# albanie/mcnCrossModalEmotions

Hardware: AMD Instinct MI355X
Metric: distillation-step samples/sec (face+audio pair) (higher is better)
Workload: dtype f32; 1 GPU; BASELINE config 4 shard: frozen resnet50 teacher fwd + VGGVox student fwd/bwd/SGD; per_gpu_batch=32, global_batch=32, face=224x224x3, teacher_batch=32, spectrogram=512x300x1, parallelism=dp1, weights=random-init (seeded), parameter_server=rccl-capi, streams=teacher one batch ahead on its own stream + wgrad side stream

## Files before the change

include/xmodal.h:

```cpp
#ifndef XMODAL_H
#define XMODAL_H
#include <stddef.h>
#ifdef __cplusplus
extern "C" {
#endif

enum {
  XM_OK = 0,
  XM_EINVAL = 1,
  XM_ENOMEM = 2,
  XM_EHIP = 3,
  XM_ETOOBIG = 4,
  XM_ENOTSUP = 5
};

enum { XM_POOL_MAX = 0, XM_POOL_AVG = 1 };
enum { XM_LOSS_SOFTMAXLOG = 0, XM_LOSS_CLASSERROR = 1 };
enum { XM_AGG_MAX = 0, XM_AGG_MEAN = 1, XM_AGG_PEAK = 2 };
enum { XM_MNR_CONVERGED = 0, XM_MNR_ITERLIMIT = 1, XM_MNR_NOTPD = 2, XM_MNR_BADINPUT = 3 };
enum { XM_ROC_OK = 0, XM_ROC_NAN = 1, XM_ROC_BADINPUT = 2 };

enum { XM_FUSE_RELU = 1, XM_BN_BATCH_MOMENTS = 2, XM_FUSE_SIGMOID = 4 };

int xm_version(void);
const char *xm_last_error(void);
int xm_device_alloc(void **ptr, size_t bytes);
int xm_device_free(void *ptr);
int xm_device_upload(void *dst_device, const void *src_host, size_t bytes);
int xm_device_download(void *dst_host, const void *src_device, size_t bytes);
int xm_device_synchronize(void);
enum { XM_EXEC_SINGLE_STREAM = 1 };
int xm_set_exec_hint(unsigned flags);
unsigned xm_get_exec_hint(void);
int xm_tune_load(const char *path);
int xm_tune_save(const char *path);
int xm_tune_entries(int *total, int *unsaved);
int xm_workspace_reserve(size_t bytes);
size_t xm_workspace_bytes(void);
int xm_workspace_reserve_stream(size_t bytes, void *stream);
unsigned long long xm_workspace_generation(void);
int xm_out_size(int in, int pad_a, int pad_b, int f, int dilate, int stride);

int xm_nnconv_forward(const float *x, int H, int W, int C, int N, const float *f, int FH, int FW,
                      int FC, int K, const float *b, float *y, int sy, int sx, int pt, int pb,
                      int pl, int pr, int dy, int dx, void *stream);
int xm_nnconv_forward_fused(const float *x, int H, int W, int C, int N, const float *f, int FH,
                            int FW, int FC, int K, const float *b, float *y, int sy, int sx,
                            int pt, int pb, int pl, int pr, int dy, int dx, const float *scale,
                            const float *shift, const float *residual, int flags, void *stream);
int xm_nnconv_forward_gated(const float *x, int H, int W, int C, int N, const float *f, int FH, int FW,
                            int FC, int K, const float *b, float *y, int sy, int sx, int pt, int pb,
                            int pl, int pr, int dy, int dx, const float *scale, const float *shift,
                            const float *gate, const float *residual, int flags, void *stream);
int xm_nnconv_forward_strided_residual(const float *x, int H, int W, int C, int N, const float *f, int FH, int FW,
                                       int FC, int K, const float *b, float *y, int sy, int sx, int pt, int pb,
                                       int pl, int pr, int dy, int dx, const float *scale, const float *shift,
                                       const float *gate, const float *residual, int res_H, int res_W, int res_sy,
                                       int res_sx, int flags, void *stream);
int xm_nnconv_forward_lattice(const float *x, int H, int W, int C, int N, const float *f, int FH, int FW, int FC, int K,
                              const float *b, float *y, int sy, int sx, int pt, int pb, int pl, int pr, int dy, int dx,
                              const float *scale, const float *shift, const float *residual, int flags, int lat_y,
                              int lat_x, void *stream);
enum { XM_CONV_F32 = 0, XM_CONV_BF16X3 = 1 };
int xm_nnconv_forward_split(const float *x, int H, int W, int C, int N, const float *f, int FH, int FW, int FC, int K,
                            const float *b, float *y, int sy, int sx, int pt, int pb, int pl, int pr, int dy, int dx,
                            const float *scale, const float *shift, const float *gate, const float *residual, int res_H,
                            int res_W, int res_sy, int res_sx, int flags, int precision, void *stream);
int xm_nnconv_split_geometry(int H, int W, int C, int N, int FH, int FW, int FC, int K, int sy, int sx, int pt, int pb,
                             int pl, int pr, int dy, int dx, int flags, int *can, int *want, int *blocks, int *launches);
int xm_nnconv_forward_moments(const float *x, int H, int W, int C, int N, const float *f, int FH, int FW,
                              int FC, int K, const float *b, float *y, int sy, int sx, int pt, int pb,
                              int pl, int pr, int dy, int dx, float epsilon, float *moments_out, void *stream);
int xm_nnconv_backward(const float *x, int H, int W, int C, int N, const float *f, int FH, int FW,
                       int FC, int K, const float *dzdy, float *dx_out, float *df_out,
                       float *db_out, int sy, int sx, int pt, int pb, int pl, int pr, int dy,
                       int dx, void *stream);
int xm_nnconv_prepare_backward(int H, int W, int C, int N, const float *f, int FH, int FW, int FC, int K,
                               int sy, int sx, int pt, int pb, int pl, int pr, int dy, int dx, void *stream);
int xm_params_changed(void);
int xm_nnconv_backward_accum(const float *x, int H, int W, int C, int N, const float *f, int FH, int FW,
                             int FC, int K, const float *dzdy, float *dx_out, float *df_out,
                             float *db_out, int sy, int sx, int pt, int pb, int pl, int pr, int dy,
                             int dx, const float *dx_accum, void *stream);
int xm_nnconv_backward_filter_bnrelupool(const float *x, int H, int W, int C, int N, int FH, int FW, int FC, int K,
                                         int sy, int sx, int pt, int pb, int pl, int pr, int dy, int dx,
                                         const float *y, const float *bn_g, const float *bn_b, const float *moments,
                                         int train, int ph, int pw, int psy, int psx, int ppt, int ppb, int ppl,
                                         int ppr, const unsigned char *argmax, const float *y_pool,
                                         const float *dzdy_pool, float *dzdf_out, float *dzdb_out, float *dg_out,
                                         float *db_out, void *stream);
int xm_nnconv_bnorm_relu_pool_forward(const float *x, int H, int W, int C, int N, const float *f, int FH, int FW, int FC,
                                      int K, const float *bias, int sy, int sx, int pt, int pb, int pl, int pr, int dy, int dx,
                                      const float *bn_g, const float *bn_b, float epsilon, const float *moments_in, int ph,
                                      int pw, int psy, int psx, int ppt, int ppb, int ppl, int ppr, double *gram,
                                      float *y_pool, unsigned char *argmax, float *moments_out, void *stream);
int xm_stem_gram(const float *x, int H, int W, int N, int FH, int FW, int sy, int sx, int pt, int pb, int pl, int pr,
                 double *gram, void *stream);
int xm_stem_gram_moments(const double *gram, const float *f, const float *b, int FH, int FW, int K, float epsilon,
                         float *moments_out, void *stream);
int xm_nnconv_backward_filter_bnrelupool_gram(const float *x, int H, int W, int C, int N, const float *f, int FH, int FW,
                                              int FC, int K, const float *bias, int sy, int sx, int pt, int pb, int pl,
                                              int pr, int dy, int dx, const float *bn_g, const float *moments, int train,
                                              int ph, int pw, int psy, int psx, int ppt, int ppb, int ppl, int ppr,
                                              const unsigned char *argmax, const float *y_pool, const float *dzdy_pool,
                                              const double *gram, float *df_out, float *dbias_out, float *dg_out,
                                              float *db_out, void *stream);

int xm_nnpool_forward(const float *x, int H, int W, int C, int N, int ph, int pw, int sy, int sx,
                      int pt, int pb, int pl, int pr, int method, float *y, void *stream);
int xm_nnpool_backward(const float *x, int H, int W, int C, int N, int ph, int pw, int sy, int sx,
                       int pt, int pb, int pl, int pr, int method, const float *dzdy, float *dx_out,
                       void *stream);

int xm_nnpool_forward_argmax(const float *x, int H, int W, int C, int N, int ph, int pw, int sy,
                             int sx, int pt, int pb, int pl, int pr, float *y, unsigned char *argmax,
                             void *stream);
int xm_nnpool_backward_argmax(const unsigned char *argmax, int H, int W, int C, int N, int ph, int pw,
                              int sy, int sx, int pt, int pb, int pl, int pr, const float *dzdy,
                              float *dx_out, void *stream);
int xm_nnpool_global_avg_backward_accum(const float *dzdy, const float *accum, float *dx_out, int H, int W, int C, int N,
                                        void *stream);

int xm_nnbnorm_forward(const float *x, int H, int W, int C, int N, const float *g, const float *b,
                       float epsilon, const float *moments_in, float *y, float *moments_out,
                       void *stream);
int xm_nnbnorm_forward_fused(const float *x, int H, int W, int C, int N, const float *g,
                             const float *b, float epsilon, const float *moments_in, float *y,
                             float *moments_out, int flags, void *stream);
int xm_nnbnorm_backward(const float *x, int H, int W, int C, int N, const float *g, const float *b,
                        const float *dzdy, float epsilon, const float *moments_in, float *dx_out,
                        float *dg_out, float *db_out, float *moments_out, void *stream);
int xm_nnbnorm_backward_fused(const float *x, const float *y, int H, int W, int C, int N,
                              const float *g, const float *b, const float *dzdy, float epsilon,
                              const float *moments_in, float *dx_out, float *dg_out, float *db_out,
                              float *moments_out, int flags, void *stream);

int xm_nnbnorm_backward_dxsum(const float *x, const float *y, int H, int W, int C, int N,
                              const float *g, const float *b, const float *dzdy, float epsilon,
                              const float *moments_in, float *dx_out, float *dg_out, float *db_out,
                              float *moments_out, float *dxsum_out, int flags, void *stream);

int xm_nnbnorm_relu_pool_forward(const float *x, int H, int W, int C, int N, const float *g,
                                 const float *b, float epsilon, const float *moments_in, int ph, int pw,
                                 int sy, int sx, int pt, int pb, int pl, int pr, float *y_pool,
                                 unsigned char *argmax, float *moments_out, void *stream);
int xm_nnbnorm_relu_pool_backward(const float *x, int H, int W, int C, int N, const float *g,
                                  const float *b, const float *moments, int train, int ph, int pw,
                                  int sy, int sx, int pt, int pb, int pl, int pr,
                                  const unsigned char *argmax, const float *y_pool, const float *dzdy_pool,
                                  float *dx_out, float *dg_out, float *db_out, float *dxsum_out, void *stream);

int xm_nnrelu(const float *x, size_t n, float leak, const float *dzdy, float *y, void *stream);
int xm_nnsigmoid(const float *x, size_t n, const float *dzdy, float *y, void *stream);
int xm_sum2(const float *a, const float *b, size_t n, int flags, float *y, void *stream);
int xm_scale_axpy(const float *x, int HW, int CN, const float *a, const float *r, int flags,
                  float *y, void *stream);
int xm_scale_backward(const float *x, int HW, int CN, const float *a, const float *dzdy,
                      float *dx_out, float *da_out, void *stream);

int xm_nndropout_forward(const float *x, size_t n, float rate, unsigned long long seed, unsigned long long offset,
                         float *y, float *mask_out, void *stream);
int xm_nndropout_apply(const float *x, const float *mask, size_t n, float *y, void *stream);

int xm_se_squeeze_bn(const float *u, int H, int W, int C, int N, const float *g, const float *b, const float *moments,
                     float *gp_out, void *stream);
int xm_scale_axpy_bn(const float *u, int H, int W, int C, int N, const float *a, const float *r, const float *g,
                     const float *b, const float *moments, int flags, float *y, void *stream);
int xm_se_tail_backward_reduce(const float *y, const float *dzdy, const float *u, int H, int W, int C, int N,
                               const float *g, const float *b, const float *moments, float *da_out, double *plane_sums,
                               void *stream);
int xm_se_tail_backward_apply(const float *y, const float *dzdy, const float *u, int H, int W, int C, int N,
                              const float *gate, const float *dgp, const float *g, const float *moments, int train,
                              const double *plane_sums, float *dz_out, float *du_out, float *dg_out, float *db_out,
                              void *stream);

int xm_nnsoftmaxt(const float *x, int HW, int C, int N, float temperature, float *y, void *stream);
int xm_nnsoftmaxt_backward(const float *x, const float *dzdy, int HW, int C, int N, float temperature,
                           float *dx, void *stream);
int xm_nnsoftmaxceloss(const float *x, const float *p, int C, int N, float temperature,
                       int logit_targets, const float *instance_weights, const float *dzdy,
                       float *y, void *stream);
#define XM_REGLOSS_EUCLIDEAN 0
#define XM_REGLOSS_HUBER 1
int xm_nnregloss(const float *x, const float *t, int E, int N, int kind, float sigma,
                 const float *instance_weights, const float *dzdy, float *y, void *stream);
int xm_nnloss(const float *x, const float *labels, int C, int N, int loss, const float *dzdy,
              float *y, void *stream);

int xm_sgd_update(float *w, float *m, const float *der, size_t n, float lr, float momentum,
                  float weight_decay, float batch, void *stream);
enum { XM_SOLVER_ADAGRAD = 0, XM_SOLVER_RMSPROP = 1, XM_SOLVER_ADADELTA = 2, XM_SOLVER_ADAM = 3, XM_SOLVER_NESTEROV = 4 };
int xm_solver_update(int kind, float *w, float *s1, float *s2, const float *der, size_t n, float lr,
                     float weight_decay, float batch, const float *coef, void *stream);
int xm_average_update(float *w, const float *der, size_t n, float lr, float denom,
                      void *stream);
int xm_scale_f32(float *x, size_t n, float a, void *stream);
int xm_comm_unique_id(void *id128);
int xm_comm_init(const void *id128, int rank, int world);
int xm_allreduce_sum_f32(float *buf, size_t n, void *stream);
int xm_parserv_push(float *buf, size_t n, void *producer_stream);
int xm_parserv_sync(void *consumer_stream);
int xm_comm_count(int *ranks);
int xm_comm_destroy(void);

int xm_spec_rownorm(const float *spec, int H, int W, int N, float *out, void *stream);
int xm_resample(const float *x, int Lx, const float *h, int Lh, int p, int q, int delay, float *y, int Ly, void *stream);
int xm_wav_batch(const float *wav, long long wav_len, const float *noise, long long noise_len, const long long *desc,
                 const float *ratio, int N, float *z, int L, void *stream);
int xm_spec_bucket_batch(const float *wav, long long wav_len, const long long *desc, int N, int rsize, const float *bank,
                         int taps, int hop, int B, float *out, void *stream);
int xm_spec_magnitude(const float *reim, int Wo, int B, int N, float *out, void *stream);
int xm_aggregate_logits(const float *frame_logits, int F_total, int E, const int *first,
                        const int *last, int N, int agg, float *out, float *max_label,
                        void *stream);
int xm_max_label(const float *x, int C, int N, float *labels, void *stream);
int xm_window_targets(const float *logits, int E, int n, const int *first, const int *last, int N, int agg, int P,
                      float *out, float *max_label, void *stream);
int xm_class_stats(const float *x, const float *labels, int C, int N, float *correct,
                   float *population, void *stream);
int xm_normalize_face(const float *rgb, int H, int W, int N, const float *avg3, float *out,
                      void *stream);
int xm_crop_resize_face(const float *src, int Hin, int Win, int N, float crop, int Ho, int Wo,
                        const float *avg3, float *out, void *stream);

int xm_mnrfit(const float *x, int p, int n, const int *labels, int k, const int *offsets, const int *rows, int nnz,
              int G, int max_iter, double tol_x, double *b_out, double *dev_out, int *iters_out, int *status_out,
              void *stream);
int xm_mnrval(const double *b, const float *x, int p, int n, int k, const int *offsets, const int *rows, int nnz, int G,
              const int *labels, double *probs_out, int *preds_out, int *conf_out, void *stream);

int xm_roc(const float *scores, int n, int E, const int *cls, const int *offsets, const int *rows, int nnz, int G,
           double *auc, long long *area, int *counts, int *status, int *perm_out, int *tp_out, void *stream);
int xm_roc_launches(void);
int xm_label_hist(const float *x, int N, int E, int sample_major, long long *bins, void *stream);

int xm_group_rows(const int *ids, int n, const int *keys, int T, int key_max, int *offsets_out, int *rows_out,
                  int *nnz_out, void *stream);
int xm_gather_rows(const float *mat, int F, int E, int row0, const int *rows, int n, float *packed, void *stream);
int xm_scatter_rows(const float *packed, int n, int E, float *mat, int F, int row0, const int *rows, void *stream);
int xm_track_peaks(const float *logits, int F, int E, const int *offsets, const int *rows, int T, int *frame_idx,
                   int *tag, float *maxed, void *stream);

int xm_nnaffinegrid(const float *A, int N, int Ho, int Wo, float *grid, void *stream);
int xm_nnaffinegrid_backward(const float *dgrid, int N, int Ho, int Wo, float *dA, void *stream);
int xm_nnbilinearsampler(const float *x, int H, int W, int C, int N, const float *grid, int Ho, int Wo, int No,
                         float *y, void *stream);
int xm_nnbilinearsampler_backward(const float *x, int H, int W, int C, int N, const float *grid, int Ho, int Wo,
                                  int No, const float *dy, float *dx, float *dgrid, void *stream);
int xm_ferplus_batch(const float *grey, int H, int W, int N, const int *flip, const float *A, int Ho, int Wo,
                     const float *avg3, float *out, void *stream);

enum { XM_JPEG_OK = 0, XM_JPEG_TRUNCATED = 1, XM_JPEG_BADCODE = 2 };
enum { XM_JPEG_DESC = 24, XM_JPEG_LANE = 4, XM_JPEG_QT_BYTES = 128, XM_JPEG_HT_BYTES = 1024, XM_JPEG_SIZES = 8 };
int xm_jpeg_plan(const unsigned char *bytes, const long long *offsets, int N, long long *desc, long long *lanes,
                 long long lanes_cap, unsigned char *tables, long long tables_cap, long long *sizes);
int xm_jpeg_decode_batch(const unsigned char *bytes, long long nbytes, const long long *desc, int N, const long long *lanes,
                         int nlanes, const unsigned char *tables, int nq, int nh, long long coef_elems,
                         long long plane_bytes, long long pixel_floats, float *pixels, float *faces, float crop, int Ho,
                         int Wo, const float *avg3, int *status, void *stream);

int xm_jpeg_decode_batch_split(const unsigned char *bytes, long long nbytes, const long long *desc, int N,
                               const long long *lanes, int nlanes, const unsigned char *tables, int nq, int nh,
                               long long coef_elems, long long plane_bytes, long long pixel_floats, float *pixels,
                               float *faces, float crop, int Ho, int Wo, const float *avg3, int *status, int seg_bytes,
                               int *rounds, void *stream);
int xm_jpeg_split_geometry(int *segments_per_pass, int *launches);

enum { XM_JPEG_SCAN = 24, XM_JPEG_PROG_SIZES = 11, XM_JPEG_MAX_SCANS = 256, XM_JPEG_MAX_LEVELS = 14 };
#define XM_JPEG_SMOOTH (1LL << 40)
enum { XM_JPEG_SCAN_SEQ = 0, XM_JPEG_SCAN_DC_FIRST = 1, XM_JPEG_SCAN_DC_REFINE = 2, XM_JPEG_SCAN_AC_FIRST = 3,
       XM_JPEG_SCAN_AC_REFINE = 4 };
int xm_jpeg_plan_prog(const unsigned char *bytes, const long long *offsets, int N, long long *desc, long long *scans,
                      long long scans_cap, long long *lanes, long long lanes_cap, unsigned char *tables, long long tables_cap,
                      long long *sizes);
int xm_jpeg_decode_batch_prog(const unsigned char *bytes, long long nbytes, const long long *desc, int N,
                              const long long *lanes, int nlanes, const unsigned char *tables, int nq, int nh,
                              long long coef_elems, long long plane_bytes, long long pixel_floats, float *pixels, float *faces,
                              float crop, int Ho, int Wo, const float *avg3, int *status, const long long *scans, int nscans,
                              int levels, int smooth, void *stream);

enum { XM_WAV_U8 = 0, XM_WAV_S16 = 1, XM_WAV_S24 = 2, XM_WAV_S32 = 3, XM_WAV_F32 = 4, XM_WAV_F64 = 5 };
enum { XM_WAV_OK = 0, XM_WAV_TRUNCATED = 1 };
enum { XM_WAV_DESC = 16, XM_WAV_SIZES = 2 };
int xm_wav_plan(const unsigned char *bytes, const long long *offsets, int N, const long long *ranges, int channel,
                long long out_base, long long *desc, long long *sizes);
int xm_wav_decode_batch(const unsigned char *bytes, long long nbytes, const long long *desc, int N, float *out,
                        long long out_floats, void *stream);

int xm_wav_plan_fs(const unsigned char *bytes, const long long *offsets, int N, const long long *ranges, int channel,
                   long long fs, long long out_base, long long *desc, long long *sizes);
int xm_wav_decode_resample_batch(const unsigned char *bytes, long long nbytes, const long long *desc, int N, float *out,
                                 long long out_floats, void *stream);
int xm_wav_resample_geometry(int *tile, int *launches);

enum { XM_PIX_DESC = 8, XM_PIX_SIZES = 2 };
enum { XM_PIX_BADCHAR = 1, XM_PIX_RANGE = 2, XM_PIX_COUNT = 4, XM_PIX_NOFIT = 8 };
int xm_pixcsv_plan(const unsigned char *bytes, long long nbytes, long long *desc, long long max_rows, long long *sizes);
int xm_pixcsv_decode_batch(const unsigned char *bytes, long long nbytes, const long long *desc, int N, int H, int W,
                           int transpose, float *out, long long out_floats, int *status, void *stream);
int xm_pixcsv_geometry(int *bytes_per_pass, int *launches);

int xm_nnnormalize_forward(const float *x, int H, int W, int C, int S, int N, float kappa, float alpha, float beta,
                           float *y, void *stream);
int xm_nnnormalize_backward(const float *x, const float *dzdy, int H, int W, int C, int S, int N, float kappa,
// ... 8 lines not shown
```

mcncrossmodalemotions_amd/_lib.py:

```python
import ctypes as C
import os

import torch

_HERE = os.path.dirname(os.path.abspath(__file__))
SO_PATH = os.environ.get("XM_LIB_PATH") or os.path.join(_HERE, "libxmodal_hip.so")

c_fp = C.c_void_p
_i, _f, _sz, _vp = C.c_int, C.c_float, C.c_size_t, C.c_void_p

SIGNATURES = {
    "xm_version": [],
    "xm_last_error": [],
    "xm_tune_load": [C.c_char_p],
    "xm_tune_save": [C.c_char_p],
    "xm_tune_entries": [C.POINTER(C.c_int), C.POINTER(C.c_int)],
    "xm_set_exec_hint": [C.c_uint],
    "xm_get_exec_hint": [],
    "xm_workspace_reserve": [_sz],
    "xm_workspace_bytes": [],
    "xm_workspace_reserve_stream": [_sz, _vp],
    "xm_workspace_generation": [],
    "xm_device_alloc": [C.POINTER(C.c_void_p), _sz],
    "xm_device_free": [_vp],
    "xm_device_upload": [_vp, _vp, _sz],
    "xm_device_download": [_vp, _vp, _sz],
    "xm_device_synchronize": [],
    "xm_out_size": [_i] * 6,
    "xm_nnconv_forward": [c_fp] + [_i] * 4 + [c_fp] + [_i] * 4 + [c_fp, c_fp] + [_i] * 8 + [_vp],
    "xm_nnconv_forward_moments": [c_fp] + [_i] * 4 + [c_fp] + [_i] * 4 + [c_fp, c_fp] + [_i] * 8 + [_f, c_fp, _vp],
    "xm_nnconv_forward_gated": [c_fp] + [_i] * 4 + [c_fp] + [_i] * 4 + [c_fp, c_fp] + [_i] * 8 +
                               [c_fp, c_fp, c_fp, c_fp, _i, _vp],
    "xm_nnconv_forward_strided_residual": [c_fp] + [_i] * 4 + [c_fp] + [_i] * 4 + [c_fp, c_fp] + [_i] * 8 +
                                          [c_fp, c_fp, c_fp, c_fp] + [_i] * 5 + [_vp],
    "xm_nnconv_forward_split": [c_fp] + [_i] * 4 + [c_fp] + [_i] * 4 + [c_fp, c_fp] + [_i] * 8 +
                               [c_fp, c_fp, c_fp, c_fp] + [_i] * 6 + [_vp],
    "xm_nnconv_split_geometry": [_i] * 17 + [C.POINTER(C.c_int)] * 4,
    "xm_nnconv_forward_lattice": [c_fp] + [_i] * 4 + [c_fp] + [_i] * 4 + [c_fp, c_fp] + [_i] * 8 +
                                 [c_fp, c_fp, c_fp, _i, _i, _i, _vp],
    "xm_nnconv_forward_fused": [c_fp] + [_i] * 4 + [c_fp] + [_i] * 4 + [c_fp, c_fp] + [_i] * 8 +
                               [c_fp, c_fp, c_fp, _i, _vp],
    "xm_nnconv_backward": [c_fp] + [_i] * 4 + [c_fp] + [_i] * 4 + [c_fp, c_fp, c_fp, c_fp] +
                          [_i] * 8 + [_vp],
    "xm_nnconv_backward_accum": [c_fp] + [_i] * 4 + [c_fp] + [_i] * 4 + [c_fp, c_fp, c_fp, c_fp] +
                                [_i] * 8 + [c_fp, _vp],
    "xm_nnconv_prepare_backward": [_i] * 4 + [c_fp] + [_i] * 12 + [_vp],
    "xm_nnconv_backward_filter_bnrelupool": [c_fp] + [_i] * 16 + [c_fp, c_fp, c_fp, c_fp] + [_i] * 9 +
                                            [c_fp, c_fp, c_fp, c_fp, c_fp, c_fp, c_fp, _vp],
    "xm_stem_gram": [c_fp] + [_i] * 11 + [_vp, _vp],
    "xm_stem_gram_moments": [_vp, c_fp, c_fp, _i, _i, _i, _f, c_fp, _vp],
    "xm_nnconv_backward_filter_bnrelupool_gram": [c_fp] + [_i] * 4 + [c_fp] + [_i] * 4 + [c_fp] + [_i] * 8 +
                                                 [c_fp, c_fp] + [_i] * 9 + [c_fp, c_fp, c_fp, _vp, c_fp, c_fp, c_fp, c_fp, _vp],
    "xm_nnconv_bnorm_relu_pool_forward": [c_fp] + [_i] * 4 + [c_fp] + [_i] * 4 + [c_fp] + [_i] * 8 + [c_fp, c_fp, _f, c_fp] +
                                         [_i] * 8 + [_vp, c_fp, c_fp, c_fp, _vp],
    "xm_params_changed": [],
    "xm_nnpool_forward": [c_fp] + [_i] * 13 + [c_fp, _vp],
    "xm_nnpool_backward": [c_fp] + [_i] * 13 + [c_fp, c_fp, _vp],
    "xm_nnpool_forward_argmax": [c_fp] + [_i] * 12 + [c_fp, c_fp, _vp],
    "xm_nnpool_backward_argmax": [c_fp] + [_i] * 12 + [c_fp, c_fp, _vp],
    "xm_nnpool_global_avg_backward_accum": [c_fp, c_fp, c_fp, _i, _i, _i, _i, _vp],
    "xm_nnbnorm_forward": [c_fp] + [_i] * 4 + [c_fp, c_fp, _f, c_fp, c_fp, c_fp, _vp],
    "xm_nnbnorm_forward_fused": [c_fp] + [_i] * 4 + [c_fp, c_fp, _f, c_fp, c_fp, c_fp, _i, _vp],
    "xm_nnbnorm_backward": [c_fp] + [_i] * 4 + [c_fp, c_fp, c_fp, _f, c_fp, c_fp, c_fp, c_fp, c_fp,
                                               _vp],
    "xm_nnbnorm_backward_fused": [c_fp, c_fp] + [_i] * 4 + [c_fp, c_fp, c_fp, _f, c_fp, c_fp, c_fp,
                                                             c_fp, c_fp, _i, _vp],
    "xm_nnbnorm_backward_dxsum": [c_fp, c_fp] + [_i] * 4 + [c_fp, c_fp, c_fp, _f, c_fp, c_fp, c_fp,
                                                             c_fp, c_fp, c_fp, _i, _vp],
    "xm_nnbnorm_relu_pool_forward": [c_fp] + [_i] * 4 + [c_fp, c_fp, _f, c_fp] + [_i] * 8 +
                                    [c_fp, c_fp, c_fp, _vp],
    "xm_nnbnorm_relu_pool_backward": [c_fp] + [_i] * 4 + [c_fp, c_fp, c_fp, _i] + [_i] * 8 +
                                     [c_fp, c_fp, c_fp, c_fp, c_fp, c_fp, c_fp, _vp],
    "xm_nndropout_forward": [c_fp, _sz, _f, C.c_ulonglong, C.c_ulonglong, c_fp, c_fp, _vp],
    "xm_nndropout_apply": [c_fp, c_fp, _sz, c_fp, _vp],
    "xm_nnrelu": [c_fp, _sz, _f, c_fp, c_fp, _vp],
    "xm_nnsigmoid": [c_fp, _sz, c_fp, c_fp, _vp],
    "xm_sum2": [c_fp, c_fp, _sz, _i, c_fp, _vp],
    "xm_scale_axpy": [c_fp, _i, _i, c_fp, c_fp, _i, c_fp, _vp],
    "xm_scale_backward": [c_fp, _i, _i, c_fp, c_fp, c_fp, c_fp, _vp],
    "xm_se_squeeze_bn": [c_fp] + [_i] * 4 + [c_fp, c_fp, c_fp, c_fp, _vp],
    "xm_scale_axpy_bn": [c_fp] + [_i] * 4 + [c_fp, c_fp, c_fp, c_fp, c_fp, _i, c_fp, _vp],
    "xm_se_tail_backward_reduce": [c_fp, c_fp, c_fp] + [_i] * 4 + [c_fp, c_fp, c_fp, c_fp, c_fp, _vp],
    "xm_se_tail_backward_apply": [c_fp, c_fp, c_fp] + [_i] * 4 + [c_fp, c_fp, c_fp, c_fp, _i, c_fp, c_fp, c_fp, c_fp, c_fp, _vp],
    "xm_nnsoftmaxt": [c_fp, _i, _i, _i, _f, c_fp, _vp],
    "xm_nnsoftmaxt_backward": [c_fp, c_fp, _i, _i, _i, _f, c_fp, _vp],
    "xm_nnregloss": [c_fp, c_fp, _i, _i, _i, _f, c_fp, c_fp, c_fp, _vp],
    "xm_nnsoftmaxceloss": [c_fp, c_fp, _i, _i, _f, _i, c_fp, c_fp, c_fp, _vp],
    "xm_nnloss": [c_fp, c_fp, _i, _i, _i, c_fp, c_fp, _vp],
    "xm_sgd_update": [c_fp, c_fp, c_fp, _sz, _f, _f, _f, _f, _vp],
    "xm_solver_update": [_i, c_fp, c_fp, c_fp, c_fp, _sz, _f, _f, _f, C.POINTER(C.c_float), _vp],
    "xm_average_update": [c_fp, c_fp, _sz, _f, _f, _vp],
    "xm_comm_unique_id": [_vp],
    "xm_comm_init": [_vp, _i, _i],
    "xm_allreduce_sum_f32": [c_fp, _sz, _vp],
    "xm_parserv_push": [c_fp, _sz, _vp],
    "xm_parserv_sync": [_vp],
    "xm_comm_count": [C.POINTER(C.c_int)],
    "xm_scale_f32": [c_fp, _sz, _f, _vp],
    "xm_comm_destroy": [],
    "xm_spec_rownorm": [c_fp, _i, _i, _i, c_fp, _vp],
    "xm_spec_magnitude": [c_fp, _i, _i, _i, c_fp, _vp],
    "xm_resample": [c_fp, _i, c_fp, _i, _i, _i, _i, c_fp, _i, _vp],
    "xm_wav_batch": [c_fp, C.c_longlong, c_fp, C.c_longlong, c_fp, c_fp, _i, c_fp, _i, _vp],
    "xm_spec_bucket_batch": [c_fp, C.c_longlong, c_fp, _i, _i, c_fp, _i, _i, _i, c_fp, _vp],
    "xm_aggregate_logits": [c_fp, _i, _i, c_fp, c_fp, _i, _i, c_fp, c_fp, _vp],
    "xm_max_label": [c_fp, _i, _i, c_fp, _vp],
    "xm_window_targets": [c_fp, _i, _i, c_fp, c_fp, _i, _i, _i, c_fp, c_fp, _vp],
    "xm_class_stats": [c_fp, c_fp, _i, _i, c_fp, c_fp, _vp],
    "xm_normalize_face": [c_fp, _i, _i, _i, C.POINTER(C.c_float), c_fp, _vp],
    "xm_crop_resize_face": [c_fp, _i, _i, _i, _f, _i, _i, C.POINTER(C.c_float), c_fp, _vp],
    "xm_nnaffinegrid": [c_fp, _i, _i, _i, c_fp, _vp],
    "xm_nnaffinegrid_backward": [c_fp, _i, _i, _i, c_fp, _vp],
    "xm_nnbilinearsampler": [c_fp] + [_i] * 4 + [c_fp] + [_i] * 3 + [c_fp, _vp],
    "xm_nnbilinearsampler_backward": [c_fp] + [_i] * 4 + [c_fp] + [_i] * 3 + [c_fp, c_fp, c_fp, _vp],
    "xm_ferplus_batch": [c_fp, _i, _i, _i, c_fp, c_fp, _i, _i, C.POINTER(C.c_float), c_fp, _vp],
    "xm_mnrfit": [c_fp, _i, _i, c_fp, _i, c_fp, c_fp, _i, _i, _i, C.c_double, c_fp, c_fp, c_fp, c_fp, _vp],
    "xm_mnrval": [c_fp, c_fp, _i, _i, _i, c_fp, c_fp, _i, _i, c_fp, c_fp, c_fp, c_fp, _vp],
    "xm_roc": [c_fp, _i, _i, c_fp, c_fp, c_fp, _i, _i, c_fp, c_fp, c_fp, c_fp, c_fp, c_fp, _vp],
    "xm_roc_launches": [],
    "xm_label_hist": [c_fp, _i, _i, _i, c_fp, _vp],
    "xm_group_rows": [c_fp, _i, c_fp, _i, _i, c_fp, c_fp, c_fp, _vp],
    "xm_gather_rows": [c_fp, _i, _i, _i, c_fp, _i, c_fp, _vp],
    "xm_scatter_rows": [c_fp, _i, _i, c_fp, _i, _i, c_fp, _vp],
    "xm_track_peaks": [c_fp, _i, _i, c_fp, c_fp, _i, c_fp, c_fp, c_fp, _vp],
    "xm_jpeg_plan": [_vp, _vp, _i, _vp, _vp, C.c_longlong, _vp, C.c_longlong, _vp],
    "xm_jpeg_decode_batch": [c_fp, C.c_longlong, c_fp, _i, c_fp, _i, c_fp, _i, _i, C.c_longlong, C.c_longlong, C.c_longlong,
                             c_fp, c_fp, _f, _i, _i, C.POINTER(C.c_float), c_fp, _vp],
    "xm_jpeg_decode_batch_split": [c_fp, C.c_longlong, c_fp, _i, c_fp, _i, c_fp, _i, _i, C.c_longlong, C.c_longlong,
                                   C.c_longlong, c_fp, c_fp, _f, _i, _i, C.POINTER(C.c_float), c_fp, _i, c_fp, _vp],
    "xm_jpeg_split_geometry": [C.POINTER(C.c_int), C.POINTER(C.c_int)],
    "xm_jpeg_plan_prog": [_vp, _vp, _i, _vp, _vp, C.c_longlong, _vp, C.c_longlong, _vp, C.c_longlong, _vp],
    "xm_jpeg_decode_batch_prog": [c_fp, C.c_longlong, c_fp, _i, c_fp, _i, c_fp, _i, _i, C.c_longlong, C.c_longlong,
                                  C.c_longlong, c_fp, c_fp, _f, _i, _i, C.POINTER(C.c_float), c_fp, c_fp, _i, _i, _i, _vp],
    "xm_wav_plan": [_vp, _vp, _i, _vp, _i, C.c_longlong, _vp, _vp],
    "xm_wav_decode_batch": [c_fp, C.c_longlong, c_fp, _i, c_fp, C.c_longlong, _vp],
    "xm_wav_plan_fs": [_vp, _vp, _i, _vp, _i, C.c_longlong, C.c_longlong, _vp, _vp],
    "xm_wav_decode_resample_batch": [c_fp, C.c_longlong, c_fp, _i, c_fp, C.c_longlong, _vp],
    "xm_wav_resample_geometry": [C.POINTER(C.c_int), C.POINTER(C.c_int)],
    "xm_pixcsv_plan": [_vp, C.c_longlong, _vp, C.c_longlong, _vp],
    "xm_pixcsv_decode_batch": [c_fp, C.c_longlong, c_fp, _i, _i, _i, _i, c_fp, C.c_longlong, c_fp, _vp],
    "xm_pixcsv_geometry": [C.POINTER(C.c_int), C.POINTER(C.c_int)],
    "xm_nnnormalize_forward": [c_fp] + [_i] * 5 + [_f, _f, _f, c_fp, _vp],
    "xm_nnnormalize_backward": [c_fp, c_fp] + [_i] * 5 + [_f, _f, _f, c_fp, _vp],
    "xm_nnnormalize_geometry": [C.POINTER(C.c_int)] * 3,
}
_RESTYPES = {"xm_get_exec_hint": C.c_uint, "xm_last_error": C.c_char_p, "xm_workspace_bytes": C.c_size_t,
             "xm_workspace_generation": C.c_ulonglong}
_DEBUG = {"xm_debug_set": [C.c_char_p, _i], "xm_debug_get": [C.c_char_p],
          "xm_prof_enable": [_i],
          "xm_prof_collect": [_i, C.POINTER(C.c_int), C.POINTER(C.c_double), C.POINTER(C.c_double),
                              C.POINTER(C.c_longlong)],
          "xm_prof_collect_bytes": [_i, C.POINTER(C.c_int), C.POINTER(C.c_double)],
          "xm_prof_kernel_name": [_i, C.c_char_p, _i]}
_SWITCHES = {"xm_debug_force_conv_cfg": "conv_cfg", "xm_debug_force_conv_splits": "conv_splits",
             "xm_debug_force_conv_halo": "conv_halo", "xm_debug_force_conv_stem": "conv_stem",
             "xm_debug_force_conv_stem3": "conv_stem3", "xm_debug_force_wgrad_patch": "wgrad_patch",
             "xm_debug_force_wgrad_patch_s2": "wgrad_patch_s2", "xm_debug_force_dgrad_s2": "dgrad_s2",
             "xm_debug_force_spec_blocks": "spec_blocks"}

_lib = None


class XmError(RuntimeError):
    def __init__(self, code, msg):
        super().__init__("xmodal error %d: %s" % (code, msg))
        self.code = code


def load():
    global _lib
    if _lib is not None:
        return _lib
    if not os.path.exists(SO_PATH):
        raise ImportError(
            "%s not found: build it with `python -m mcncrossmodalemotions_amd.build` "
            "(hipcc --offload-arch=gfx950); there is no CPU fallback" % SO_PATH)
    lib = C.CDLL(SO_PATH, mode=C.RTLD_GLOBAL)
    for name, args in list(SIGNATURES.items()) + list(_DEBUG.items()):
        fn = getattr(lib, name)
        fn.argtypes = args
        fn.restype = _RESTYPES.get(name, C.c_int)
    for name, key in _SWITCHES.items():
        setattr(lib, name, (lambda k: (lambda v: lib.xm_debug_set(k, int(v))))(key.encode()))
    lib.xm_debug_num_conv_cfgs = lambda: lib.xm_debug_get(b"num_conv_cfgs")
    lib.xm_debug_comm_force_single = lambda v: 0 if lib.xm_debug_set(b"comm_single", int(v)) > -2 else 1
    if hasattr(lib, "xm_debug_conv_cycles"):
        lib.xm_debug_conv_cycles.argtypes = [_i, C.POINTER(C.c_ulonglong), _i]
        lib.xm_debug_conv_cycles.restype = C.c_int
    _lib = lib
    return lib


def check(rc):
    if rc != 0:
        raise XmError(rc, load().xm_last_error().decode("utf-8", "replace"))
```

mcncrossmodalemotions_amd/build.py:

```python
import os
import subprocess
import sys
from concurrent.futures import ThreadPoolExecutor

HERE = os.path.dirname(os.path.abspath(__file__))
CSRC = os.path.join(HERE, "csrc")
TAG = os.environ.get("XM_BUILD_TAG", "")
OUT = os.path.join(HERE, "libxmodal_hip%s.so" % ("_" + TAG if TAG else ""))
SOURCES = ["context.cpp", "prof.cpp", "conv.hip", "conv_split.hip", "stem_pool.hip", "norm_pool.hip", "lrn.hip", "misc.hip", "spec.hip", "sampler.hip", "eval.hip", "roc.hip", "imdb.hip", "jpeg.hip", "jpeg_prog.hip", "wav.hip", "pixcsv.hip", "comm.cpp"]
HEADERS = ["xm_common.h", "fastdiv.h", "prof.h", "conv_plan.h", "stem_pool_plan.h", "conv_split_plan.h", "norm_pool_plan.h", "conv_tune.h", "wav_plan.h", "wav_resample.h", "pixcsv_plan.h", "jpeg_scan_plan.h", "jpeg_entropy.h", "conv_kernels.h", "stem_pool_kernels.h", os.path.join("..", "..", "include", "xmodal.h")]
FLAGS = ["--offload-arch=gfx950", "-O3", "-std=c++17", "-fPIC", "-Wall", "-Wno-unused-function"]
if os.environ.get("XM_DEBUG_CYCLES"):
    FLAGS.append("-DXM_DEBUG_CYCLES")
FLAGS += os.environ.get("XM_DEFINES", "").split()


def _stale(target, deps):
    if not os.path.exists(target):
        return True
    t = os.path.getmtime(target)
    return any(os.path.getmtime(d) > t for d in deps)


def build(force=False, verbose=False):
    hipcc = os.environ.get("HIPCC", "/opt/rocm/bin/hipcc")
    objdir = os.path.join(CSRC, "_obj" + ("_" + TAG if TAG else ""))
    os.makedirs(objdir, exist_ok=True)
    hdrs = [os.path.join(CSRC, h) for h in HEADERS]
    jobs = []
    objs = []
    for s in SOURCES:
        src = os.path.join(CSRC, s)
        obj = os.path.join(objdir, s + ".o")
        objs.append(obj)
        if force or _stale(obj, [src] + hdrs):
            jobs.append([hipcc] + FLAGS + ["-x", "hip", "-c", src, "-o", obj])

    def run(cmd):
        if verbose:
            print(" ".join(cmd), file=sys.stderr)
        subprocess.check_call(cmd)

    if jobs:
        with ThreadPoolExecutor(max_workers=min(len(jobs), os.cpu_count() or 4)) as ex:
            list(ex.map(run, jobs))
    if jobs or force or _stale(OUT, objs):
        run([hipcc, "--offload-arch=gfx950", "-shared", "-fPIC", "-o", OUT] + objs +
            ["-L/opt/rocm/lib", "-lrccl", "-Wl,-rpath,/opt/rocm/lib"])
    return OUT


if __name__ == "__main__":
    print(build(force="--force" in sys.argv, verbose=True))
```

mcncrossmodalemotions_amd/csrc/context.cpp:

```cpp
#include <cstdlib>
#include <map>
#include <string>
#include <vector>

#include "xm_common.h"

namespace xm {
bool path_on(Path p) {
  static const char *const kEnv[kPathCount] = {"XM_NO_HYBRID",      "XM_NO_HALO",        "XM_NO_SKINNY",     "XM_NO_SKINNY4",
                                               "XM_NO_STEM",        "XM_NO_STEM_WGRAD",  "XM_NO_DMA",        "XM_NO_FUSED_STATS",
                                               "XM_DGRAD_MERGE",    "XM_NO_FAST_TRANSPOSE", "XM_NO_POOL_LDS", "XM_NO_POOL_PATCH",
                                               "XM_NO_POOL_POOLED", "XM_NO_W8", "XM_NO_WGRAD_PATCH", "XM_NO_WGRAD_PATCH_S2", "XM_NO_DGRAD_S2", "XM_NO_STEM3"};
  static bool on[kPathCount];
  static bool read = false;
  if (!read) {
    for (int i = 0; i < kPathCount; ++i) on[i] = getenv(kEnv[i]) == nullptr;
    read = true;
  }
  return on[p];
}

long long env_int(const char *name, long long dflt) {
  const char *e = getenv(name);
  return (e && *e) ? atoll(e) : dflt;
}
double env_double(const char *name, double dflt) {
  const char *e = getenv(name);
  return (e && *e) ? atof(e) : dflt;
}

static char g_err[512] = "";
char *err_buf() { return g_err; }

int fail(int code, const char *fmt, ...) {
  va_list ap;
  va_start(ap, fmt);
  vsnprintf(g_err, sizeof g_err, fmt, ap);
  va_end(ap);
  return code;
}

struct WsBuf {
  void *ptr = nullptr;
  size_t cap = 0;
};
static std::map<hipStream_t, WsBuf> g_ws;
static unsigned long long g_ws_generation = 0;

int ws_get(size_t bytes, void **ptr, hipStream_t stream) {
  WsBuf &w = g_ws[stream];
  if (bytes > w.cap) {
    size_t want = bytes + bytes / 4 + (1u << 20);
    static const bool verbose = getenv("XM_WS_VERBOSE") != nullptr;
    if (verbose) fprintf(stderr, "[xm ws] stream %p grow %zu -> %zu\n", (void *)stream, w.cap, want);
    ++g_ws_generation;
    if (w.ptr) {
      hipError_t e = hipDeviceSynchronize();
      if (e != hipSuccess) return fail(XM_EHIP, "hipDeviceSynchronize -> %s", hipGetErrorString(e));
      (void)hipFree(w.ptr);
      w.ptr = nullptr;
      w.cap = 0;
    }
    hipError_t e = hipMalloc(&w.ptr, want);
    if (e != hipSuccess) {
      w.ptr = nullptr;
      return fail(XM_ENOMEM, "workspace hipMalloc(%zu) -> %s", want, hipGetErrorString(e));
    }
    w.cap = want;
  }
  *ptr = w.ptr;
  return XM_OK;
}

static std::map<std::string, void *> g_tables;

const void *cached_device_table(const void *host, size_t bytes) {
  std::string key((const char *)host, bytes);
  auto it = g_tables.find(key);
  if (it != g_tables.end()) return it->second;
  void *d = nullptr;
  static const bool verbose = getenv("XM_WS_VERBOSE") != nullptr;
  if (verbose) fprintf(stderr, "[xm ws] new device table %zu bytes (#%zu)\n", bytes, g_tables.size());
  if (hipMalloc(&d, bytes) != hipSuccess) return nullptr;
  if (hipMemcpy(d, host, bytes, hipMemcpyHostToDevice) != hipSuccess) {
    (void)hipFree(d);
    return nullptr;
  }
  g_tables.emplace(std::move(key), d);
  return d;
}

}

extern "C" {

int xm_version(void) { return 124; }
const char *xm_last_error(void) { return xm::err_buf(); }

int xm_workspace_reserve(size_t bytes) {
  void *p;
  return xm::ws_get(bytes, &p, nullptr);
}
int xm_workspace_reserve_stream(size_t bytes, void *stream) {
  void *p;
  return xm::ws_get(bytes, &p, (hipStream_t)stream);
}
unsigned long long xm_workspace_generation(void) { return xm::g_ws_generation; }

int xm_device_alloc(void **ptr, size_t bytes) {
  if (!ptr) return xm::fail(XM_EINVAL, "device_alloc: NULL output");
  *ptr = nullptr;
  if (bytes == 0) return XM_OK;
  hipError_t e = hipMalloc(ptr, bytes);
  if (e != hipSuccess) return xm::fail(XM_ENOMEM, "hipMalloc(%zu) -> %s", bytes, hipGetErrorString(e));
  return XM_OK;
}
int xm_device_free(void *ptr) {
  if (!ptr) return XM_OK;
  hipError_t e = hipFree(ptr);
  if (e != hipSuccess) return xm::fail(XM_EHIP, "hipFree -> %s", hipGetErrorString(e));
  return XM_OK;
}
int xm_device_upload(void *dst_device, const void *src_host, size_t bytes) {
  if (bytes == 0) return XM_OK;
  if (!dst_device || !src_host) return xm::fail(XM_EINVAL, "device_upload: NULL pointer");
  hipError_t e = hipMemcpy(dst_device, src_host, bytes, hipMemcpyHostToDevice);
  if (e != hipSuccess) return xm::fail(XM_EHIP, "hipMemcpy(H2D, %zu) -> %s", bytes, hipGetErrorString(e));
  return XM_OK;
}
int xm_device_download(void *dst_host, const void *src_device, size_t bytes) {
  if (bytes == 0) return XM_OK;
  if (!dst_host || !src_device) return xm::fail(XM_EINVAL, "device_download: NULL pointer");
  hipError_t e = hipMemcpy(dst_host, src_device, bytes, hipMemcpyDeviceToHost);
  if (e != hipSuccess) return xm::fail(XM_EHIP, "hipMemcpy(D2H, %zu) -> %s", bytes, hipGetErrorString(e));
  return XM_OK;
}
int xm_device_synchronize(void) {
  hipError_t e = hipDeviceSynchronize();
  if (e != hipSuccess) return xm::fail(XM_EHIP, "hipDeviceSynchronize -> %s", hipGetErrorString(e));
  return XM_OK;
}
size_t xm_workspace_bytes(void) {
  size_t t = 0;
  for (auto &kv : xm::g_ws) t += kv.second.cap;
  return t;
}

int xm_out_size(int in, int pad_a, int pad_b, int f, int dilate, int stride) {
  return xm::out_size(in, pad_a, pad_b, f, dilate, stride);
}
}
```

mcncrossmodalemotions_amd/csrc/conv.hip:

```cpp
#include <dlfcn.h>

#include <algorithm>
#include <climits>
#include <cstdlib>
#include <map>
#include <string>
#include <vector>

#include "conv_kernels.h"
#include "conv_tune.h"
#include "prof.h"

namespace xm {


__global__ void pad_filter_kernel(const float *__restrict__ f, float *__restrict__ o, int M, int R,
                                  int Rp) {
  size_t i = blockIdx.x * (size_t)blockDim.x + threadIdx.x;
  if (i >= (size_t)M * Rp) return;
  int r = (int)(i % Rp);
  size_t m = i / Rp;
  o[i] = r < R ? f[m * R + r] : 0.f;
}

// ... 969 lines not shown
  a.A = f, a.lda = R, a.nbm = 1, a.nbn = (a.NP + 127) / 128, a.slab = nullptr;
  a.hyS = 1, a.hyFull = 0, a.hyTps = 0, a.hyP0 = 0, a.piReal = 0;
  a.dbgCycles = g_dbg_cycles;
  const double abytes = (double)a.xBytes + 4.0 * a.M * a.Rtrue + 4.0 * a.M * (double)a.NP;
  ProfScope ps(prof_key(kProfStem), 2.0 * a.M * (double)a.NP * a.Rtrue, st, abytes);
  const int grid = stem_grid(a.NP);
  if (a.gsy == 2) hipLaunchKernelGGL(conv_stem_kernel<2>, dim3(grid), dim3(256), 0, st, a, a.nbn);
  else hipLaunchKernelGGL(conv_stem_kernel<1>, dim3(grid), dim3(256), 0, st, a, a.nbn);
  XM_LAUNCH_CHECK();
  return XM_OK;
}

static int g_force_stem3 = -1;
static bool stem3_ok(const ConvGemmArgs &a, const Geo &g, const float *x, bool stats) {
  if (!path_on(kPathStem3) || forced_tiling()) return false;
  if (!stem3_can(g, (uintptr_t)x, epilogue_flags(a, stats))) return false;
  return g_force_stem3 == 1 || fills_chip(g);
}
static int launch_stem3(ConvGemmArgs a, const float *f, int R, hipStream_t st) {
  a.A = f, a.lda = R, a.nbm = 1, a.nbn = a.NP / 128, a.slab = nullptr;
  const double abytes = (double)a.xBytes + 4.0 * a.M * a.Rtrue + 4.0 * a.M * (double)a.NP;
  static const bool wide_on = env_int("XM_STEM3_WIDE", 1) != 0;
  const int pij = (int)a.divPIJ.d, pi = (int)a.divPI.d;
  const bool wide = wide_on && pij % 256 == 0 && pi >= 86;
  if (wide) a.nbn = a.NP / 256;
  ProfScope ps(prof_key(kProfStem3, wide ? 1 : 0), 2.0 * a.M * (double)a.NP * a.Rtrue, st, abytes);
  const int grid = std::min(512, (a.nbn + 7) / 8 * 8);
  if (wide) hipLaunchKernelGGL(conv_stem3_kernel<2>, dim3(grid), dim3(256), 0, st, a, a.nbn);
  else hipLaunchKernelGGL(conv_stem3_kernel<1>, dim3(grid), dim3(256), 0, st, a, a.nbn);
  XM_LAUNCH_CHECK();
  return XM_OK;
}

static size_t slab_floats(int M, int NP, int Rp, int ncfg, int nU, int nV, int Rtrue) {
  ConvGemmArgs proto{};
  proto.M = M, proto.NP = NP, proto.Rp = Rp;
  size_t need = 0;
  for (int c = 0; c < ncfg; ++c) {
    int sp;
    need = std::max(need, gemm_slab_floats(proto, c, &sp));
  }
  if (nU <= 3 && nV <= 3 && nU * nV >= 4 && Rtrue % (kHaloCB * nU * nV) == 0) {
    proto.Rtrue = Rtrue, proto.nU = nU, proto.nV = nV;
    need = std::max(need, halo_slab_floats(proto));
  }
  return need;
}

struct FwdOperands {
  const float *x, *A, *b, *scale, *shift, *resid, *gate;
  float *y;
  const int2 *taps;
  int lda, Rp, relu;
  bool bigTaps, dma_ok;
  int rH = 0, rW = 0, rsy = 1, rsx = 1;
  bool resid_strided(const Geo &g) const { return resid && (rH != g.Ho || rW != g.Wo || rsy != 1 || rsx != 1); }
};

static ConvGemmArgs forward_args(const Geo &g, int grp, const FwdOperands &o) {
  ConvGemmArgs a{};
  const size_t xoff = (size_t)grp * g.FC * g.H * g.W, yoff = (size_t)grp * g.Kg * g.Ho * g.Wo;
  a.A = o.A + (size_t)grp * g.Kg * o.lda, a.lda = o.lda, a.aBytes = (unsigned)((size_t)g.Kg * o.lda * 4);
  a.X = o.x + xoff, a.xBytes = (unsigned)((x_elements(g) - xoff) * 4), a.xSampleStride = g.H * g.W * g.C;
  a.Y = o.y + yoff, a.taps = o.taps, a.tapStride = (unsigned)((size_t)g.H * g.W * 4);
  a.bias = o.b ? o.b + grp * g.Kg : nullptr;
  a.scale = o.scale ? o.scale + grp * g.Kg : nullptr, a.shift = o.shift ? o.shift + grp * g.Kg : nullptr;
  a.resid = o.resid ? o.resid + yoff : nullptr, a.relu = o.relu;
  if (o.resid_strided(g)) {
    a.resid = o.resid + (size_t)grp * g.Kg * o.rH * o.rW;
    a.rsOn = 1, a.rsy = o.rsy, a.rsx = o.rsx, a.rH = o.rH;
    a.rChanStride = o.rH * o.rW, a.rSampleStride = o.rH * o.rW * g.K;
  }
  a.gate = o.gate ? o.gate + (size_t)grp * g.Kg : nullptr, a.gateStride = g.K;
  a.M = g.Kg, a.Rp = o.Rp, a.Rtrue = g.R;
  a.PI = g.Ho, a.PJ = g.Wo, a.NP = g.Ho * g.Wo * g.N;
  a.divPIJ = make_fastdiv((uint32_t)(g.Ho * g.Wo)), a.divPI = make_fastdiv((uint32_t)g.Ho);
  a.gsy = g.sy, a.gsx = g.sx, a.gh0 = -g.pt, a.gw0 = -g.pl, a.LimH = g.H, a.LimW = g.W;
  a.nU = o.bigTaps ? 1 : g.FH, a.nV = o.bigTaps ? 1 : g.FW;
  a.du0 = 0, a.dus = g.dy, a.dv0 = 0, a.dvs = g.dx;
  a.osy = 1, a.osx = 1, a.oh0 = 0, a.ow0 = 0, a.OH = g.Ho;
  a.oChanStride = g.Ho * g.Wo, a.oSampleStride = g.Ho * g.Wo * g.K, a.divMU = make_fastdiv(1), a.oUStride = 0;
  a.vecStore = ((g.Ho * g.Wo) % 4 == 0 && (((uintptr_t)a.Y | (a.rsOn ? 0 : (uintptr_t)a.resid)) & 15) == 0) ? 1 : 0;
  a.dmaOk = (o.dma_ok && a.vecStore && !a.rsOn) ? 1 : 0;
  return a;
}

struct FwdStats {
  bool ok;
  float *part;
  int ncg;
};
static ConvGemmArgs stats_args(const ConvGemmArgs &a, FwdStats &s, int ncg) {
  ConvGemmArgs aa = a;
  s.ncg = ncg;
  if (ncg > 0) aa.statPart = s.part, aa.statNcg = ncg;
  return aa;
}
static int forward_stats_reduce(const FwdStats &s, double *part2, float *moments_out, int K, int NP, float eps, hipStream_t st) {
  const int S = std::max(1, std::min(64, s.ncg / 768));
  g_last_stats_splits = S;
  hipLaunchKernelGGL(conv_stats_reduce_kernel, dim3((K + 7) / 8, S), dim3(256), 0, st, s.part, moments_out, part2, K, s.ncg, S,
                     (double)NP, eps);
  XM_LAUNCH_CHECK();
  if (S > 1) {
    hipLaunchKernelGGL(conv_stats_finalize2_kernel, dim3((K + 255) / 256), dim3(256), 0, st, part2, moments_out, K, S,
                       (double)NP, eps);
    XM_LAUNCH_CHECK();
  }
  return XM_OK;
}

static int forward_run(const Geo &g, const ConvGemmArgs &a, const float *x, const float *f, int mode, float *slab,
                       FwdStats &s, hipStream_t st) {
  auto gemm = [&](int ci) {
    int sp;
    ci = a.dmaOk ? ci : base_cfg(ci);
    gemm_slab_floats(a, ci, &sp);
    const bool carry = s.ok && sp == 1 && g_force_splits <= 1;
    ConvGemmArgs aa = stats_args(a, s, carry ? (a.NP + kCfgs[ci].bn() - 1) / kCfgs[ci].bn() : 0);
    const int rc_ = launch_gemm(aa, mode, ci, sp, slab, st);
    if (aa.statPart) s.ncg = aa.statNcg;
    return rc_;
  };
  const TuneKey key = tune_key_forward(0, g, a.M, a.NP, a.Rp, mode + (s.ok ? 4 : 0));
  const int ci = tune_cfg(key, pick_cfg(a.M, a.NP, a.Rp / kBK), st, gemm, a.dmaOk ? kNumCfg : kNumBaseCfg, w8_skip(a.M, a.NP));
  if (!a.rsOn && stem_ok(a, g, x, s.ok)) {
    auto arm = [&](int h) { return h ? launch_stem(stats_args(a, s, s.ok ? stem_grid(a.NP) : 0), f, g.R, st) : gemm(ci); };
    return arm(select_arm(7, key, st, 2, kOneChallenger, kHaloMargin, g_force_stem, arm));
  }
  if (!a.rsOn && stem3_ok(a, g, x, s.ok)) {
    auto arm = [&](int h) { return h ? launch_stem3(a, f, g.R, st) : gemm(ci); };
    return arm(select_arm(12, key, st, 2, kOneChallenger, kHaloMargin, g_force_stem3, arm));
  }
  ConvGemmArgs ah = a;
  const int hneed = (forced_tiling() || a.rsOn) ? 0 : halo_setup(ah, g.N);
  const bool hok[4] = {true, halo_var_ok(ah, hneed, 0), halo_var_ok(ah, hneed, 1), halo_var_ok(ah, hneed, 2)};
  auto arm = [&](int h) {
    if (!h) return gemm(ci);
    const bool carry = s.ok && halo_splits(ah, h - 1) == 1;
    return launch_halo(stats_args(ah, s, carry ? (a.NP + 127) / 128 : 0), h - 1, slab, st);
  };
  return arm(select_arm(4, key, st, 4, hok, kHaloMargin, halo_forced(hok), arm));
}

static bool fwd_dma_ok(const Geo &g, const float *x, const float *f, bool need_pad, int mode) {
  return !need_pad && mode == 0 && g.FH == 1 && g.FW == 1 && g.sy == 1 && g.sx == 1 && g.dy == 1 &&
         g.dx == 1 && (g.H * g.W) % 4 == 0 && ((uintptr_t)x & 15) == 0 && ((uintptr_t)f & 15) == 0 &&
         g.R % kBK == 0 && path_on(kPathDma);
}

static int conv_forward(const float *x, const float *f, const float *b, float *y, const Geo &g,
                        const float *scale, const float *shift, const float *resid, int relu,
                        hipStream_t st, float *moments_out = nullptr, float eps = 0.f, const float *gate = nullptr,
                        int res_H = 0, int res_W = 0, int res_sy = 1, int res_sx = 1) {
  const bool padded = (g.pt | g.pb | g.pl | g.pr) != 0;
  const bool bigTaps = g.FH * g.FW > 63;
  if (bigTaps && padded)
    return fail(XM_ENOTSUP, "vl_nnconv: padded filters with more than 63 spatial taps (%dx%d) are not built",
                g.FH, g.FW);
  const int Rp = (g.R + kBK - 1) / kBK * kBK;
  const bool need_pad = (g.R % kBK) != 0 || ((uintptr_t)f & 15);
  const int mode = (padded || Rp != g.R) ? 1 : 0;
  const int NP = g.Ho * g.Wo * g.N;
  const size_t slabf = slab_floats(g.Kg, NP, Rp, kNumCfg, g.FH, g.FW, g.R);
  const bool dma_ok = fwd_dma_ok(g, x, f, need_pad, mode);
  const bool want_stats = moments_out != nullptr && g.G == 1 && path_on(kPathFusedStats);
  const size_t statf = want_stats ? (size_t)2 * g.K * std::max((NP + 31) / 32, stem_grid(NP)) : 0;
  const size_t stat2 = want_stats ? (size_t)2 * g.K * 64 : 0;
  WsCarver ws;
  int rc = ws.init(WsCarver::need(need_pad ? (size_t)g.K * Rp : 0, 4) + WsCarver::need(slabf, 4) +
                       WsCarver::need(statf, 4) + WsCarver::need(stat2, 8), st);
  if (rc) return rc;
  FwdOperands o{x, f, b, scale, shift, resid, gate, y, device_taps(fwd_tap_table(g, Rp, bigTaps)), g.R, Rp, relu, bigTaps, dma_ok};
  if (!o.taps) return fail(XM_ENOMEM, "vl_nnconv: tap table allocation failed");
  if (resid) o.rH = res_H > 0 ? res_H : g.Ho, o.rW = res_W > 0 ? res_W : g.Wo, o.rsy = res_sy, o.rsx = res_sx;
  if (need_pad) {
    float *Ap = ws.take<float>((size_t)g.K * Rp);
    size_t n = (size_t)g.K * Rp;
    hipLaunchKernelGGL(pad_filter_kernel, dim3((unsigned)((n + 255) / 256)), dim3(256), 0, st, f, Ap,
                       g.K, g.R, Rp);
    XM_LAUNCH_CHECK();
    o.A = Ap;
    o.lda = Rp;
  }
  float *slab = slabf ? ws.take<float>(slabf) : nullptr;
  float *statp = statf ? ws.take<float>(statf) : nullptr;
  double *statp2 = stat2 ? ws.take<double>(stat2) : nullptr;
  bool stats_done = false;
  if (moments_out) g_last_stats_splits = 0;
  for (int grp = 0; grp < g.G; ++grp) {
    ConvGemmArgs a = forward_args(g, grp, o);
    FwdStats s{want_stats && a.vecStore && !relu && !resid, statp, 0};
    if (s.ok) a.dmaOk = 0;
    rc = forward_run(g, a, x, f, mode, slab, s, st);
    if (rc) return rc;
    if (s.ncg > 0) {
      rc = forward_stats_reduce(s, statp2, moments_out, g.K, NP, eps, st);
      if (rc) return rc;
      stats_done = true;
    }
  }
  if (moments_out && !stats_done) return bn_batch_moments(y, g.Ho, g.Wo, g.K, g.N, eps, moments_out, st);
  return XM_OK;
}

struct FullExtentPlan {
  int ci;
  int tps;
  int hyS, hyTps, hyP0;
};
static int g_last_lattice = 0;

static bool full_extent_plan(const Geo &g, const ConvGemmArgs &a, const float *x, int mode, bool have_slab, hipStream_t st,
                             FullExtentPlan &p) {
  if (stem_ok(a, g, x, false) || stem3_ok(a, g, x, false)) return false;
  const TuneKey key = tune_key_forward(0, g, a.M, a.NP, a.Rp, mode);
  int ci = pick_cfg(a.M, a.NP, a.Rp / kBK);
  const int ncfg = a.dmaOk ? kNumCfg : kNumBaseCfg;
  if (g_force_cfg >= 0) ci = g_force_cfg < ncfg ? g_force_cfg : base_cfg(g_force_cfg);
  else if (tune_must_measure(key, st, &ci)) return false;
  ConvGemmArgs ah = a;
  const int hneed = forced_tiling() ? 0 : halo_setup(ah, g.N);
  const bool hok[4] = {true, halo_var_ok(ah, hneed, 0), halo_var_ok(ah, hneed, 1), halo_var_ok(ah, hneed, 2)};
  if (hok[1] || hok[2] || hok[3]) {
    int arm = halo_forced(hok);
    if (arm < 0) {
      TuneKey k4 = key;
      k4.kind = 4;
      arm = 0;
      if (tune_must_measure(k4, st, &arm)) return false;
      if (arm < 0 || arm >= 4 || !hok[arm]) arm = 0;
    }
    if (arm != 0) return false;
  }
  ci = a.dmaOk ? ci : base_cfg(ci);
  int sp;
  gemm_slab_floats(a, ci, &sp);
  if (ci == kCfgW8 && !path_on(kPathW8)) ci = 0;
  const Cfg &c = kCfgs[ci];
  ConvGemmArgs t = a;
  t.nbm = (a.M + c.bm() - 1) / c.bm(), t.nbn = (a.NP + c.bn() - 1) / c.bn(), t.nkt = a.Rp / kBK;
  t.statPart = nullptr;
  p.tps = (t.nkt + sp - 1) / sp;
  p.hyS = 1, p.hyTps = 0, p.hyP0 = 0;
  if (p.tps >= t.nkt && have_slab) {
    int full;
    const int hyS = hybrid_plan(t, ci, &full);
    if (hyS > 1) {
      p.hyTps = (t.nkt + hyS - 1) / hyS;
      p.hyS = (t.nkt + p.hyTps - 1) / p.hyTps;
      p.hyP0 = full / t.nbm * c.bn();
    }
  }
  p.ci = !is_dma_cfg(ci) ? ci : (kCfgs[ci].tm * kCfgs[ci].tn == 1 ? 3 : base_cfg(ci));
  return true;
}

static int launch_gemm_lattice(ConvGemmArgs a, int mode, int ci, int tps, float *slab, int p0, hipStream_t st) {
  const Cfg &c = kCfgs[ci];
  a.nbm = (a.M + c.bm() - 1) / c.bm();
  a.nbn = (a.NP + c.bn() - 1) / c.bn();
  a.nkt = a.Rp / kBK;
  a.tilesPerSplit = std::min(tps, a.nkt);
  const int splits = (a.nkt + a.tilesPerSplit - 1) / a.tilesPerSplit;
  a.NPs = (a.NP + 3) & ~3;
  a.slab = splits > 1 ? slab : nullptr;
  a.dbgCycles = g_dbg_cycles;
  a.hyS = 1, a.hyFull = 0, a.hyTps = 0, a.hyP0 = 0;
  if (splits > 1 && !slab) return fail(XM_EINVAL, "vl_nnconv(lattice): split launch without a slab");
  {
    const double abytes = (double)a.xBytes + 4.0 * a.M * a.Rtrue + 4.0 * a.M * (double)a.NP;
    ProfScope ps(prof_key(kProfGemm, ci * 2 + mode), 2.0 * a.M * (double)a.NP * a.Rtrue, st, abytes);
    const dim3 grid(a.nbm * a.nbn, splits);
    if (mode) launch_gemm_cfg<1>(ci, a, grid, st);
    else launch_gemm_cfg<0>(ci, a, grid, st);
  }
  XM_LAUNCH_CHECK();
  g_last_combine = 0;
  if (splits > 1) {
    a.slab += p0, a.hyP0 = p0;
    launch_splitk_epilogue(a, splits, a.NP - p0, false, st);
    g_last_combine = -splits;
    XM_LAUNCH_CHECK();
  }
  return XM_OK;
}

static int conv_forward_lattice(const float *x, const float *f, const float *b, float *y, const Geo &g, const float *scale,
                                const float *shift, int relu, int ly, int lx, hipStream_t st, int *ran) {
  *ran = 0;
  const bool padded = (g.pt | g.pb | g.pl | g.pr) != 0;
  const bool bigTaps = g.FH * g.FW > 63;
  if (bigTaps && padded) return XM_OK;
  if (g.G != 1) return XM_OK;
  const int Rp = (g.R + kBK - 1) / kBK * kBK;
  const bool need_pad = (g.R % kBK) != 0 || ((uintptr_t)f & 15);
  const int mode = (padded || Rp != g.R) ? 1 : 0;
  const int NP = g.Ho * g.Wo * g.N;
  const bool have_slab = slab_floats(g.Kg, NP, Rp, kNumCfg, g.FH, g.FW, g.R) > 0;
  const int PI = lattice_extent(g.Ho, ly), PJ = lattice_extent(g.Wo, lx), NPl = PI * PJ * g.N;
  FwdOperands o{x, f, b, scale, shift, nullptr, nullptr, y, nullptr, g.R, Rp, relu, bigTaps, fwd_dma_ok(g, x, f, need_pad, mode)};
  FullExtentPlan p;
  if (!full_extent_plan(g, forward_args(g, 0, o), x, mode, have_slab, st, p)) return XM_OK;
  const int nkt = Rp / kBK;
  const int z = p.hyS > 1 ? p.hyS : (nkt + p.tps - 1) / p.tps;
  const long long cut = p.hyS > 1 ? lattice_pixels_below(p.hyP0, g.Ho, g.Wo, ly, lx) : 0;
  const int n0 = (int)(cut / (PI * PJ));
  const int NPz = NPl - n0 * PI * PJ;
  const size_t slabf = z > 1 ? (size_t)z * g.Kg * ((NPz + 3) & ~3) : 0;
  WsCarver ws;
  int rc = ws.init(WsCarver::need(need_pad ? (size_t)g.K * Rp : 0, 4) + WsCarver::need(slabf, 4), st);
  if (rc) return rc;
  o.taps = device_taps(fwd_tap_table(g, Rp, bigTaps));
  if (!o.taps) return fail(XM_ENOMEM, "vl_nnconv: tap table allocation failed");
  if (need_pad) {
    float *Ap = ws.take<float>((size_t)g.K * Rp);
    const size_t n = (size_t)g.K * Rp;
    hipLaunchKernelGGL(pad_filter_kernel, dim3((unsigned)((n + 255) / 256)), dim3(256), 0, st, f, Ap, g.K, g.R, Rp);
    XM_LAUNCH_CHECK();
    o.A = Ap;
    o.lda = Rp;
  }
  float *slab = slabf ? ws.take<float>(slabf) : nullptr;
  for (int grp = 0; grp < g.G; ++grp) {
    ConvGemmArgs a = forward_args(g, grp, o);
    a.PI = PI, a.PJ = PJ, a.NP = NPl;
    a.divPIJ = make_fastdiv((uint32_t)(PI * PJ)), a.divPI = make_fastdiv((uint32_t)PI);
    a.gsy = g.sy * ly, a.gsx = g.sx * lx;
    a.osy = ly, a.osx = lx;
    a.vecStore = 0, a.dmaOk = 0;
    if (p.hyS <= 1) {
      rc = launch_gemm_lattice(a, mode, p.ci, p.tps, slab, 0, st);
      if (rc) return rc;
      continue;
    }
    if (cut > 0) {
      ConvGemmArgs a1 = a;
      a1.NP = (int)cut;
      rc = launch_gemm_lattice(a1, mode, p.ci, nkt, nullptr, 0, st);
      if (rc) return rc;
    }
    if (cut < NPl) {
      ConvGemmArgs a2 = a;
      const size_t xskip = (size_t)n0 * g.H * g.W * g.C;
      a2.X += xskip, a2.xBytes -= (unsigned)(xskip * 4), a2.Y += (size_t)n0 * a.oSampleStride;
      a2.NP = NPz;
      rc = launch_gemm_lattice(a2, mode, p.ci, p.hyTps, slab, (int)(cut - (long long)n0 * PI * PJ), st);
      if (rc) return rc;
    }
  }
  *ran = 1;
  return XM_OK;
}

struct PrepKey {
// ... 561 lines not shown
    *s->value = s->normalise(value);
    return old;
  }
  if (key && strcmp(key, "comm_single") == 0) return comm_force_single(value);
  return INT_MIN;
}
int xm_debug_get(const char *key) {
  if (key && strcmp(key, "num_conv_cfgs") == 0) return kNumCfg;
  if (key && strcmp(key, "conv_last_combine") == 0) return g_last_combine;
  if (key && strcmp(key, "conv_last_lattice") == 0) return g_last_lattice;
  if (key && strcmp(key, "wgrad_last_splits") == 0) return g_last_wgrad_splits;
  if (key && strcmp(key, "bias_grad_last_splits") == 0) return g_last_bias_splits;
  if (key && strcmp(key, "stats_last_splits") == 0) return g_last_stats_splits;
  if (key && strcmp(key, "dgrad_last_transpose") == 0) return g_last_dgrad_transpose;
  if (key && strcmp(key, "dgrad_last_prepared") == 0) return g_last_dgrad_prepared;
  const DebugSwitch *s = debug_switch(key);
  return s ? *s->value : INT_MIN;
}

int xm_set_exec_hint(unsigned flags) {
  if (flags & ~(unsigned)XM_EXEC_SINGLE_STREAM) return fail(XM_EINVAL, "xm_set_exec_hint: unknown flag bits 0x%x", flags);
  g_exec_hint = flags;
  return XM_OK;
}
unsigned xm_get_exec_hint(void) { return g_exec_hint; }


int xm_tune_load(const char *path) {
  return g_tune.load(path && path[0] ? path : tune_default_path().c_str());
}
int xm_tune_save(const char *path) {
  tune_load_once();
  const std::string p = path && path[0] ? std::string(path) : tune_default_path();
  const int rc = g_tune.save(p.c_str());
  if (rc == 1) return fail(XM_EINVAL, "xm_tune_save: cannot write %s.tmp", p.c_str());
  if (rc) return fail(XM_EINVAL, "xm_tune_save: rename to %s failed", p.c_str());
  return XM_OK;
}
int xm_tune_entries(int *total, int *unsaved) {
  tune_load_once();
  if (total) *total = g_tune.size();
  if (unsaved) *unsaved = g_tune.unsaved;
  return XM_OK;
}
#ifdef XM_DEBUG_CYCLES
int xm_debug_conv_cycles(int on, unsigned long long *out, int nblocks) {
  const size_t bytes = 4096 * 4 * sizeof(unsigned long long);
  if (on && !g_dbg_cycles) {
    if (hipMalloc((void **)&g_dbg_cycles, bytes) != hipSuccess) return XM_ENOMEM;
    (void)hipMemset(g_dbg_cycles, 0, bytes);
  }
  if (out && g_dbg_cycles)
    (void)hipMemcpy(out, g_dbg_cycles, (size_t)std::min(nblocks, 4096) * 32, hipMemcpyDeviceToHost);
  if (!on && g_dbg_cycles) {
    (void)hipFree(g_dbg_cycles);
    g_dbg_cycles = nullptr;
  }
  return XM_OK;
}
#endif

static int fused_forward(const float *x, int H, int W, int C, int N, const float *f, int FH, int FW,
                         int FC, int K, const float *b, float *y, int sy, int sx, int pt, int pb,
                         int pl, int pr, int dy, int dx, const float *scale, const float *shift,
                         const float *gate, const float *residual, int res_H, int res_W, int res_sy,
                         int res_sx, int flags, void *stream) {
  Geo g;
  int rc = make_geo(g, H, W, C, N, FH, FW, FC, K, sy, sx, pt, pb, pl, pr, dy, dx);
  if (rc) return rc;
  if (res_H == 0) res_H = g.Ho, res_W = g.Wo, res_sy = res_sx = 1;
  if (!x || !f || !y) return fail(XM_EINVAL, "vl_nnconv: NULL tensor");
  if ((scale == nullptr) != (shift == nullptr))
    return fail(XM_EINVAL, "vl_nnconv(fused): scale and shift must be given together");
  if ((flags & XM_FUSE_RELU) && (flags & XM_FUSE_SIGMOID))
    return fail(XM_EINVAL, "vl_nnconv(fused): relu and sigmoid are exclusive");
  if (gate && (flags & XM_FUSE_SIGMOID)) return fail(XM_ENOTSUP, "vl_nnconv(gated): sigmoid epilogue is not built");
  if (residual) {
    if (res_sy < 1 || res_sx < 1 || res_H < 1 || res_W < 1 || g.Ho != (res_H - 1) / res_sy + 1 ||
        g.Wo != (res_W - 1) / res_sx + 1)
      return fail(XM_EINVAL, "vl_nnconv(fused): a %d x %d residual sampled with stride [%d %d] does not give the %d x %d output",
                  res_H, res_W, res_sy, res_sx, g.Ho, g.Wo);
    if ((long long)res_H * res_W * g.K * g.N >= (1LL << 30))
      return fail(XM_ETOOBIG, "vl_nnconv(fused): residual with >= 2^30 elements (4 GiB)");
  }
  hipStream_t st = (hipStream_t)stream;
  if (!gate && !residual && fc_skinny_ok(g))
    return fc_skinny_forward(x, f, b, y, g, (flags & XM_FUSE_SIGMOID) ? 2 : ((flags & XM_FUSE_RELU) ? 1 : 0), st, scale,
                             shift);
  rc = conv_forward(x, f, b, y, g, scale, shift, residual, (flags & XM_FUSE_RELU) ? 1 : 0, st, nullptr, 0.f, gate, res_H,
                    res_W, res_sy, res_sx);
  if (rc || !(flags & XM_FUSE_SIGMOID)) return rc;
  return xm_nnsigmoid(y, (size_t)g.Ho * g.Wo * g.K * g.N, nullptr, y, stream);
}

int xm_nnconv_forward_fused(const float *x, int H, int W, int C, int N, const float *f, int FH,
                            int FW, int FC, int K, const float *b, float *y, int sy, int sx,
                            int pt, int pb, int pl, int pr, int dy, int dx, const float *scale,
                            const float *shift, const float *residual, int flags, void *stream) {
  return fused_forward(x, H, W, C, N, f, FH, FW, FC, K, b, y, sy, sx, pt, pb, pl, pr, dy, dx, scale, shift, nullptr, residual,
                       0, 0, 1, 1, flags, stream);
}

int xm_nnconv_forward_strided_residual(const float *x, int H, int W, int C, int N, const float *f, int FH, int FW,
                                       int FC, int K, const float *b, float *y, int sy, int sx, int pt, int pb,
                                       int pl, int pr, int dy, int dx, const float *scale, const float *shift,
                                       const float *gate, const float *residual, int res_H, int res_W, int res_sy,
                                       int res_sx, int flags, void *stream) {
  if (residual && res_H < 1) return fail(XM_EINVAL, "vl_nnconv(fused): residual extent must be positive");
  return fused_forward(x, H, W, C, N, f, FH, FW, FC, K, b, y, sy, sx, pt, pb, pl, pr, dy, dx, scale, shift, gate, residual,
                       residual ? res_H : 0, res_W, res_sy, res_sx, flags, stream);
}

int xm_nnconv_forward_lattice(const float *x, int H, int W, int C, int N, const float *f, int FH, int FW, int FC, int K,
                              const float *b, float *y, int sy, int sx, int pt, int pb, int pl, int pr, int dy, int dx,
                              const float *scale, const float *shift, const float *residual, int flags, int lat_y,
                              int lat_x, void *stream) {
  Geo g;
  int rc = make_geo(g, H, W, C, N, FH, FW, FC, K, sy, sx, pt, pb, pl, pr, dy, dx);
  if (rc) return rc;
  if (!x || !f || !y) return fail(XM_EINVAL, "vl_nnconv: NULL tensor");
  if (lat_y < 1 || lat_x < 1) return fail(XM_EINVAL, "vl_nnconv(lattice): the lattice steps must be >= 1, got [%d %d]", lat_y, lat_x);
  if ((scale == nullptr) != (shift == nullptr))
    return fail(XM_EINVAL, "vl_nnconv(fused): scale and shift must be given together");
  if (residual) return fail(XM_ENOTSUP, "vl_nnconv(lattice): a residual operand is not built");
  if (flags & ~XM_FUSE_RELU) return fail(XM_ENOTSUP, "vl_nnconv(lattice): only the ReLU epilogue is built");
  g_last_lattice = 0;
  int ran = 0;
  if ((lat_y > 1 || lat_x > 1) && !fc_skinny_ok(g)) {
    rc = conv_forward_lattice(x, f, b, y, g, scale, shift, (flags & XM_FUSE_RELU) ? 1 : 0, lat_y, lat_x, (hipStream_t)stream, &ran);
    if (rc) return rc;
  }
  g_last_lattice = ran;
  if (ran) return XM_OK;
  return fused_forward(x, H, W, C, N, f, FH, FW, FC, K, b, y, sy, sx, pt, pb, pl, pr, dy, dx, scale, shift, nullptr, nullptr, 0, 0,
                       1, 1, flags, stream);
}

int xm_nnconv_forward_moments(const float *x, int H, int W, int C, int N, const float *f, int FH, int FW,
                              int FC, int K, const float *b, float *y, int sy, int sx, int pt, int pb,
                              int pl, int pr, int dy, int dx, float epsilon, float *moments_out, void *stream) {
  Geo g;
  int rc = make_geo(g, H, W, C, N, FH, FW, FC, K, sy, sx, pt, pb, pl, pr, dy, dx);
  if (rc) return rc;
  if (!x || !f || !y || !moments_out) return fail(XM_EINVAL, "vl_nnconv(+moments): NULL tensor");
  hipStream_t st = (hipStream_t)stream;
  if (fc_skinny_ok(g)) {
    g_last_stats_splits = 0;
    rc = fc_skinny_forward(x, f, b, y, g, 0, st);
    return rc ? rc : bn_batch_moments(y, g.Ho, g.Wo, g.K, g.N, epsilon, moments_out, st);
  }
  return conv_forward(x, f, b, y, g, nullptr, nullptr, nullptr, 0, st, moments_out, epsilon);
}

int xm_nnconv_forward_gated(const float *x, int H, int W, int C, int N, const float *f, int FH, int FW,
                            int FC, int K, const float *b, float *y, int sy, int sx, int pt, int pb,
                            int pl, int pr, int dy, int dx, const float *scale, const float *shift,
                            const float *gate, const float *residual, int flags, void *stream) {
  if (!gate) return fail(XM_EINVAL, "vl_nnconv(gated): NULL tensor");
  return fused_forward(x, H, W, C, N, f, FH, FW, FC, K, b, y, sy, sx, pt, pb, pl, pr, dy, dx, scale, shift, gate, residual,
                       0, 0, 1, 1, flags, stream);
}

int xm_nnconv_forward(const float *x, int H, int W, int C, int N, const float *f, int FH, int FW,
                      int FC, int K, const float *b, float *y, int sy, int sx, int pt, int pb,
                      int pl, int pr, int dy, int dx, void *stream) {
  return xm_nnconv_forward_fused(x, H, W, C, N, f, FH, FW, FC, K, b, y, sy, sx, pt, pb, pl, pr, dy,
                                 dx, nullptr, nullptr, nullptr, 0, stream);
}

int xm_nnconv_prepare_backward(int H, int W, int C, int N, const float *f, int FH, int FW, int FC, int K,
                               int sy, int sx, int pt, int pb, int pl, int pr, int dy, int dx, void *stream) {
  Geo g;
  int rc = make_geo(g, H, W, C, N, FH, FW, FC, K, sy, sx, pt, pb, pl, pr, dy, dx);
  if (rc) return rc;
  if (!f) return fail(XM_EINVAL, "vl_nnconv: F is NULL");
  return conv_dgrad(f, nullptr, nullptr, g, (hipStream_t)stream, nullptr, true);
}

int xm_params_changed(void) {
  ++g_param_version;
  return XM_OK;
}

int xm_nnconv_backward_filter_bnrelupool(const float *x, int H, int W, int C, int N, int FH, int FW, int FC, int K, int sy,
                                         int sx, int pt, int pb, int pl, int pr, int dy, int dx, const float *y,
                                         const float *bn_g, const float *bn_b, const float *moments, int train, int ph,
                                         int pw, int psy, int psx, int ppt, int ppb, int ppl, int ppr,
                                         const unsigned char *argmax, const float *y_pool, const float *dzdy_pool,
                                         float *df_out, float *dbias_out, float *dg_out, float *db_out, void *stream) {
  Geo g;
  int rc = make_geo(g, H, W, C, N, FH, FW, FC, K, sy, sx, pt, pb, pl, pr, dy, dx);
  if (rc) return rc;
  if (!x || !y || !bn_g || !bn_b || !moments || !argmax || !dzdy_pool || !df_out)
    return fail(XM_EINVAL, "vl_nnconv(filter derivative through bnorm+relu+pool): NULL tensor");
  hipStream_t st = (hipStream_t)stream;
  const int pHo = out_size(g.Ho, ppt, ppb, ph, 1, psy), pWo = out_size(g.Wo, ppl, ppr, pw, 1, psx);
  const bool ok = g_force_stem != 0 && stem_wgrad_can(g, (uintptr_t)x, (uintptr_t)y) && g.K == g.Kg && y_pool != nullptr &&
                  pool3x3s2_unpadded(ph, pw, psy, psx, ppt, ppb, ppl, ppr) && (g.Ho & 1) == 0 && pHo >= 1 && pWo >= 1 &&
                  (!dbias_out || g.R < 64) && fits_i32_bytes((size_t)pHo * pWo * g.K * g.N);
  if (!ok)
    return fail(XM_ENOTSUP, "vl_nnconv(filter derivative through bnorm+relu+pool): geometry not covered by the fused kernel");
  const int grid = stem_grid(g.Ho * g.Wo * g.N);
  WsCarver ws;
  rc = ws.init(WsCarver::need((size_t)6 * g.K, 4) + WsCarver::need((size_t)grid * 96 * 64, 4) + bnpool_sums_need(g.K, g.N), st);
  if (rc) return rc;
  float *rowc = ws.take<float>((size_t)6 * g.K);
  float *spart = ws.take<float>((size_t)grid * 96 * 64);
  rc = bnpool_backward_sums(ws, y, g.Ho, g.Wo, g.K, g.N, bn_g, bn_b, moments, train, ph, pw, psy, psx, ppt, ppb, ppl, ppr,
                            argmax, y_pool, dzdy_pool, dg_out, db_out, rowc, st);
  if (rc) return rc;
  StemBnp bnp{dzdy_pool, argmax, rowc, pHo, pWo, dbias_out};
  return launch_stem_wgrad(x, y, df_out, g, spart, grid, st, &bnp);
}

int xm_nnconv_backward(const float *x, int H, int W, int C, int N, const float *f, int FH, int FW,
                       int FC, int K, const float *dzdy, float *dx_out, float *df_out,
                       float *db_out, int sy, int sx, int pt, int pb, int pl, int pr, int dy,
                       int dx, void *stream) {
  return xm_nnconv_backward_accum(x, H, W, C, N, f, FH, FW, FC, K, dzdy, dx_out, df_out, db_out, sy, sx, pt,
                                  pb, pl, pr, dy, dx, nullptr, stream);
}

int xm_nnconv_backward_accum(const float *x, int H, int W, int C, int N, const float *f, int FH, int FW,
                             int FC, int K, const float *dzdy, float *dx_out, float *df_out,
                             float *db_out, int sy, int sx, int pt, int pb, int pl, int pr, int dy,
                             int dx, const float *dx_accum, void *stream) {
  Geo g;
  int rc = make_geo(g, H, W, C, N, FH, FW, FC, K, sy, sx, pt, pb, pl, pr, dy, dx);
  if (rc) return rc;
  if (!dzdy) return fail(XM_EINVAL, "vl_nnconv: DZDY is NULL in backward mode");
  hipStream_t st = (hipStream_t)stream;
  if (db_out) {
    int S = std::max(1, std::min(N, 2048 / K));
    if ((long long)g.Ho * g.Wo < 1024) S = 1;
    WsCarver ws;
    rc = ws.init(WsCarver::need((size_t)K * S, 8), st);
    if (rc) return rc;
    double *part = ws.take<double>((size_t)K * S);
    const int HWo = g.Ho * g.Wo;
    const bool vec = (HWo & 3) == 0 && ((uintptr_t)dzdy & 15) == 0;
    g_last_bias_splits = S;
    hipLaunchKernelGGL(bias_grad_partial_kernel, dim3(K, S), dim3(256), 0, st, dzdy, part, HWo, K, N, S, vec ? 1 : 0,
                       make_fastdiv((uint32_t)(vec ? HWo >> 2 : HWo)));
    XM_LAUNCH_CHECK();
    hipLaunchKernelGGL(bias_grad_finalize_kernel, dim3((K + 3) / 4), dim3(256), 0, st, part, db_out,
                       K, S);
    XM_LAUNCH_CHECK();
  }
  if (df_out) {
    if (!x) return fail(XM_EINVAL, "vl_nnconv: X is NULL but DZDF requested");
    rc = conv_wgrad(x, dzdy, df_out, g, st);
    if (rc) return rc;
  }
  if (dx_out) {
    if (!f) return fail(XM_EINVAL, "vl_nnconv: F is NULL but DZDX requested");
    if (dx_accum == dx_out) return fail(XM_EINVAL, "vl_nnconv: dx_accum must not alias dx_out");
    rc = conv_dgrad(f, dzdy, dx_out, g, st, dx_accum);
    if (rc) return rc;
  }
  return XM_OK;
}
}
```

mcncrossmodalemotions_amd/csrc/prof.cpp:

```cpp
#include "prof.h"

#include <algorithm>
#include <vector>

#include "xm_common.h"

namespace xm {

bool g_prof_on = false;
static std::vector<ProfRec> g_prof;
static std::vector<hipEvent_t> g_event_pool;

static hipEvent_t prof_event() {
  if (!g_event_pool.empty()) {
    hipEvent_t e = g_event_pool.back();
    g_event_pool.pop_back();
    return e;
  }
  hipEvent_t e;
  (void)hipEventCreate(&e);
  return e;
}
void prof_begin(ProfRec &r, hipStream_t st) {
  r.start = prof_event();
  r.stop = prof_event();
  (void)hipEventRecord(r.start, st);
}
void prof_end(const ProfRec &r, hipStream_t st) {
  (void)hipEventRecord(r.stop, st);
  g_prof.push_back(r);
}

struct ProfRow {
  ProfKind kind;
  int nsub;
  const char *names[6];
};
static const ProfRow kProfRows[] = {
    {kProfGemm, 2 * 12, {}},
    {kProfWgrad, 4 * 7, {}},
    {kProfGemmMulti, 2 * 8, {}},
    {kProfHalo, 3, {"conv_halo_kernel<2, 2, 2, 2, 512>", "conv_halo_kernel<3, 1, 1, 4, 512>", "conv_halo_kernel<3, 1, 1, 4, 1024>"}},
    {kProfHaloMulti, 3, {"conv_halo_multi_kernel<2, 2, 2, 2, 512>", "conv_halo_multi_kernel<3, 1, 1, 4, 512>",
                         "conv_halo_multi_kernel<3, 1, 1, 4, 1024>"}},
    {kProfStem, 1, {"conv_stem_kernel<2>"}},
    {kProfStemWgrad, 2, {"conv_stem_wgrad_kernel<2>", "conv_stem_wgrad_bnp_kernel<2, 2>"}},
    {kProfWgradPatch, 1, {"conv_wgrad_patch_kernel<30>"}},
    {kProfWgradPatchS2, 1, {"conv_wgrad_patch_s2_kernel<5, 2>"}},
    {kProfDgradS2, 1, {"conv_dgrad_s2_kernel<1>"}},
    {kProfStem3, 2, {"conv_stem3_kernel<1>", "conv_stem3_kernel<2>"}},
    {kProfStemGram, 1, {"stem_gram_kernel<2>"}},
    {kProfStemWgradPool, 2, {"conv_stem_wgrad_pool_kernel<2, false>", "conv_stem_wgrad_pool_kernel<2, true>"}},
    {kProfStemBnpoolFwd, 1, {"conv_stem_bnpool_fwd_kernel"}},
    {kProfSpec, 4, {"spec_bank_kernel", "spec_plan_kernel", "spec_gemm_kernel", "spec_finish_kernel"}},
    {kProfJpeg, 6, {"jpeg_clear_kernel", "jpeg_entropy_kernel", "jpeg_idct_kernel", "jpeg_colour_kernel",
                    "crop_resize_face_ragged_kernel", "jpeg_entropy_split_kernel"}},
    {kProfJpegProg, 3, {"jpeg_entropy_prog_kernel", "jpeg_smooth_kernel", "jpeg_smooth_dc_kernel"}},
    {kProfWav, 1, {"wav_decode_kernel"}},
    {kProfWavRate, 2, {"wav_rate_gain_kernel", "wav_resample_kernel"}},
    {kProfPixcsv, 1, {"pixcsv_decode_kernel"}},
    {kProfConvSplit, 1, {"conv_split_kernel"}},
    {kProfLrn, 6, {"lrn_forward_kernel<5, false>", "lrn_forward_kernel<5, true>", "lrn_backward_kernel<5, false>",
                   "lrn_backward_kernel<5, true>", "lrn_general_kernel<false>", "lrn_general_kernel<true>"}},
};

static size_t prof_slot(std::vector<int> &ks, int key) {
  const size_t i = std::find(ks.begin(), ks.end(), key) - ks.begin();
  if (i == ks.size()) ks.push_back(key);
  return i;
}

}

using namespace xm;

extern "C" {

int xm_prof_enable(int on) {
  if (on) {
    for (auto &r : g_prof) {
      g_event_pool.push_back(r.start);
      g_event_pool.push_back(r.stop);
    }
    g_prof.clear();
  }
  g_prof_on = on != 0;
  return XM_OK;
}

int xm_prof_collect(int cap, int *keys, double *total_ms, double *total_flops, long long *launches) {
  std::vector<int> ks;
  std::vector<double> ms, fl;
  std::vector<long long> cnt;
  for (auto &r : g_prof) {
    float t = 0.f;
    if (hipEventElapsedTime(&t, r.start, r.stop) != hipSuccess) continue;
    const size_t i = prof_slot(ks, r.key);
    if (i == ms.size()) ms.push_back(0), fl.push_back(0), cnt.push_back(0);
    ms[i] += t;
    fl[i] += r.flops;
    cnt[i] += 1;
  }
  for (size_t i = 0; i < ks.size() && (int)i < cap; ++i) {
    keys[i] = ks[i];
    total_ms[i] = ms[i];
    total_flops[i] = fl[i];
    launches[i] = cnt[i];
  }
  return (int)ks.size();
}

int xm_prof_collect_bytes(int cap, int *keys, double *total_bytes) {
  std::vector<int> ks;
  std::vector<double> by;
  for (auto &r : g_prof) {
    const size_t i = prof_slot(ks, r.key);
    if (i == by.size()) by.push_back(0);
    by[i] += r.bytes;
  }
  for (size_t i = 0; i < ks.size() && (int)i < cap; ++i) {
    keys[i] = ks[i];
    total_bytes[i] = by[i];
  }
  return (int)ks.size();
}

int xm_prof_kernel_name(int key, char *buf, int len) {
  if (!buf || len <= 0) return fail(XM_EINVAL, "xm_prof_kernel_name: no buffer");
  buf[0] = 0;
  const int kind = key / 100, sub = key % 100;
  for (const ProfRow &row : kProfRows) {
    if (key < 0 || kind != row.kind || sub >= row.nsub) continue;
    if (row.names[0]) {
      snprintf(buf, len, "%s", row.names[sub]);
      return XM_OK;
    }
    if (conv_cfg_kernel_name(row.kind, sub, buf, len)) return XM_OK;
  }
  return fail(XM_EINVAL, "xm_prof_kernel_name: no launch site records key %d", key);
}

}
```

mcncrossmodalemotions_amd/csrc/prof.h:

```cpp
#pragma once
#include <hip/hip_runtime.h>

namespace xm {

enum ProfKind {
  kProfGemm = 0,
  kProfWgrad = 1,
  kProfGemmMulti = 2,
  kProfHalo = 3,
  kProfHaloMulti = 4,
  kProfStem = 5,
  kProfStemWgrad = 6,
  kProfWgradPatch = 9,
  kProfWgradPatchS2 = 10,
  kProfDgradS2 = 11,
  kProfStem3 = 12,
  kProfStemGram = 13,
  kProfStemWgradPool = 14,
  kProfStemBnpoolFwd = 15,
  kProfSpec = 20,
  kProfJpeg = 21,
  kProfWav = 22,
  kProfPixcsv = 23,
  kProfLrn = 25,
  kProfJpegProg = 26,
  kProfWavRate = 27,
  kProfConvSplit = 28,
};
constexpr int prof_key(ProfKind kind, int sub = 0) { return kind * 100 + sub; }

struct ProfRec {
  hipEvent_t start, stop;
  int key;
  double flops;
  double bytes;
};
extern bool g_prof_on;
void prof_begin(ProfRec &r, hipStream_t st);
void prof_end(const ProfRec &r, hipStream_t st);

struct ProfScope {
  const bool on;
  ProfRec r;
  hipStream_t st;
  ProfScope(int key, double flops, hipStream_t s, double bytes = 0) : on(g_prof_on), st(s) {
    if (!on) return;
    r.key = key;
    r.flops = flops;
    r.bytes = bytes;
    prof_begin(r, st);
  }
  ~ProfScope() { if (on) prof_end(r, st); }
};

bool conv_cfg_kernel_name(ProfKind kind, int sub, char *buf, int len);

}
```

mcncrossmodalemotions_amd/csrc/xm_common.h:

```cpp
#pragma once
#include <hip/hip_runtime.h>

#include <cstdarg>
#include <cstdint>
#include <cstdio>
#include <cstring>

#include "../../include/xmodal.h"
#include "fastdiv.h"

namespace xm {

char *err_buf();
int fail(int code, const char *fmt, ...);

#define XM_HIP(expr)                                                                  \
  do {                                                                                \
    hipError_t e__ = (expr);                                                          \
    if (e__ != hipSuccess)                                                            \
      return xm::fail(XM_EHIP, "%s -> %s (%s:%d)", #expr, hipGetErrorString(e__), __FILE__, __LINE__); \
  } while (0)

#define XM_LAUNCH_CHECK()                                                             \
  do {                                                                                \
    hipError_t e__ = hipGetLastError();                                               \
    if (e__ != hipSuccess)                                                            \
      return xm::fail(XM_EHIP, "kernel launch -> %s (%s:%d)", hipGetErrorString(e__), __FILE__, __LINE__); \
  } while (0)

int ws_get(size_t bytes, void **ptr, hipStream_t stream);
struct WsCarver {
  char *base = nullptr;
  size_t off = 0, cap = 0;
  int init(size_t bytes, hipStream_t stream) {
    void *p = nullptr;
    int rc = ws_get(bytes, &p, stream);
    base = (char *)p;
    cap = bytes;
    off = 0;
    return rc;
  }
  template <class T>
  T *take(size_t count) {
    size_t b = (count * sizeof(T) + 255) & ~size_t(255);
    T *p = (T *)(base + off);
    off += b;
    return p;
  }
  static size_t need(size_t count, size_t elt) { return (count * elt + 255) & ~size_t(255); }
};

enum Path {
  kPathHybrid,
  kPathHalo,
  kPathSkinny,
  kPathSkinny4,
  kPathStem,
  kPathStemWgrad,
  kPathDma,
  kPathFusedStats,
  kPathDgradMerge,
  kPathFastTranspose,
  kPathPoolLds,
  kPathPoolPatch,
  kPathPoolPooled,
  kPathW8,
  kPathWgradPatch,
  kPathWgradPatchS2,
  kPathDgradS2,
  kPathStem3,
  kPathCount
};
bool path_on(Path p);
long long env_int(const char *name, long long dflt);
double env_double(const char *name, double dflt);

int comm_force_single(int on);
extern int g_spec_blocks;
extern int g_conv_split_want;
extern int g_force_stem;
struct Geo;
int make_geo(Geo &g, int H, int W, int C, int N, int FH, int FW, int FC, int K, int sy, int sx, int pt, int pb, int pl,
             int pr, int dy, int dx);

const void *cached_device_table(const void *host, size_t bytes);

int bn_batch_moments(const float *x, int H, int W, int C, int N, float eps, float *moments_out, hipStream_t st);

size_t bnpool_sums_need(int C, int N);
int bnpool_backward_sums(WsCarver &ws, const float *x, int H, int W, int C, int N, const float *g, const float *b,
                         const float *moments, int train, int ph, int pw, int sy, int sx, int pt, int pb, int pl, int pr,
                         const unsigned char *amax, const float *y_pool, const float *dzdy_pool, float *dg_out,
                         float *db_out, float *rowc_out, hipStream_t st);

int face_ragged_launch(const float *pixels, const long long *desc, int stride, int col_h, int col_w, int col_pix, int N,
                       float crop, int Ho, int Wo, const float *avg3, float *out, hipStream_t st);

static inline int out_size(int in, int pa, int pb, int f, int d, int s) {
  int feff = (f - 1) * d + 1;
  int t = in + pa + pb - feff;
  return t < 0 ? 0 : t / s + 1;
}

static inline bool too_big(long long a, long long b = 1, long long c = 1, long long d = 1) {
  return a * b * c * d >= (1LL << 31);
}

#ifdef __HIPCC__
typedef float f32x16 __attribute__((ext_vector_type(16)));
typedef float f32x4 __attribute__((ext_vector_type(4)));
#endif

}

#ifdef __HIPCC__
__device__ __forceinline__ uint32_t xm_div(uint32_t n, const xm::FastDiv f) {
  return xm::fast_div(n, f);
}
__device__ __forceinline__ float xm_wave_sum(float v) {
#pragma unroll
  for (int o = 32; o > 0; o >>= 1) v += __shfl_xor(v, o, 64);
  return v;
}
__device__ __forceinline__ double xm_wave_sum_d(double v) {
#pragma unroll
  for (int o = 32; o > 0; o >>= 1) v += __shfl_xor(v, o, 64);
  return v;
}
__device__ __forceinline__ float xm_wave_max(float v) {
#pragma unroll
  for (int o = 32; o > 0; o >>= 1) v = fmaxf(v, __shfl_xor(v, o, 64));
  return v;
}
#endif
```

mcncrossmodalemotions_amd/dagnn.py:

```python
import os
from collections import OrderedDict

import numpy as np
import torch

from . import vl


class Param:
    def __init__(self, name, value=None, learningRate=1.0, weightDecay=1.0, trainMethod="gradient"):
        self.name = name
        self.value = value
        self.der = None
        self.learningRate = learningRate
        self.weightDecay = weightDecay
        self.trainMethod = trainMethod
        self.fanout = 0


class Var:
    def __init__(self, name):
        self.name = name
        self.value = None
        self.der = None
# ... 640 lines not shown
                for v in step.reads:
                    ev = pending.pop(v, None)
                    if ev is not None:
                        torch.cuda.current_stream().wait_event(ev)
            step.forward(self)
        mark("fwd1")
        if derOutputs is None:
            return
        for k, d in derOutputs.items():
            if not isinstance(d, torch.Tensor):
                cache = self._der_consts
                key = (float(d), str(self.device))
                if key not in cache:
                    cache[key] = vl.from_numpy(np.array([[float(d)]], np.float32), self.device)
                d = cache[key]
            self.vars[k].der = d
        if not self.accumulateParamDers and self._flat is None:
            for p in self.params.values():
                p.der = None
        self._pending_param_ders = {}
        hooks = self.bwdHooks
        for step in reversed(plan):
            if hooks:
                h = hooks.get(step.rec.name)
                if h is not None:
                    h()
            step.backward(self)
        mark("bwd1")
        if self._side_pending:
            torch.cuda.current_stream().wait_stream(self.wgradStream)
            self._side_pending = False
        mark("join")

    def _set_var_der(self, name, d):
        if d is None:
            return
        v = self.vars[name]
        if v.der is None:
            v.der = d
        else:
            v.der = vl.sum2(v.der, d)

    def _direct_der(self, rec):
        if self._flat is None or self.accumulateParamDers:
            return None
        ps = [self.params[p] for p in rec.params]
        if any(p.fanout > 1 or p.der is None for p in ps):
            return None
        return [p.der for p in ps]

    def _set_param_der(self, name, d):
        if d is None:
            return
        p = self.params[name]
        if self._flat is not None and d is p.der:
            return
        seen = self._pending_param_ders.get(name, 0)
        self._pending_param_ders[name] = seen + 1
        if self._flat is not None:
            if seen == 0 and not self.accumulateParamDers:
                p.der.copy_(d)
            else:
                p.der.add_(d)
        else:
            p.der = d if (p.der is None or seen == 0 and not self.accumulateParamDers) else vl.sum2(p.der, d)

    def _plan(self, training):
        if self.convPrecision not in ("fp32", "bf16x3"):
            raise ValueError("dagnn: convPrecision is %r, expected 'fp32' or 'bf16x3'" % (self.convPrecision,))
        key = (training, self.mode, self.fuse, self.stridePrune, self.latticePrune, self.convPrecision, len(self.layers),
               tuple(n for n, v in self.vars.items() if v.precious))
        layers = [id(l) for l in self.layers]
        if self._plan_key != key or self._plan_layers != layers:
            self._plan_key, self._plan_layers, self._plan_cache = key, layers, build_plan(self, training)
        return self._plan_cache


def load_mat(path):
    from . import matfile
    return matfile.load_mat(path)


def save_mat(net, path, wrap=None):
    from . import matfile
    return matfile.save_mat(net, path, wrap)


class FlatParams:
    def __init__(self, val, der, mom, segments):
        self.val, self.der, self.mom, self.segments = val, der, mom, segments
        self.state2 = None
        self.solver_t = None


def _release_der(net, var):
    if net.conserveMemory and not var.precious:
        var.der = None


class _Step:

    reads_through_conv = False

    def __init__(self, rec, *swallowed):
        self.rec = rec
        self.recs = [rec] + [q for q in swallowed if q is not None]
        self.outputs = self.recs[-1].outputs
        made = {v for q in self.recs for v in q.outputs}
        self.reads = tuple(dict.fromkeys(v for q in self.recs for v in q.inputs if v not in made))
        self.run_stride = None
        self.out_lattice = None
        self.precision = None
        self._split_ok = {}

    def _stride(self):
        return self.rec.block.stride if self.run_stride is None else self.run_stride

    def _params(self, net):
        return [net.params[p].value for p in self.rec.params]

    def _values(self, net, ins):
        return self.rec.block.forward(ins, self._params(net))

    def _derivatives(self, net, ins, douts):
        return self.rec.block.backward(ins, self._params(net), douts)

    def forward(self, net):
        outs = self._values(net, [net.vars[v].value for v in self.rec.inputs])
        for v, t in zip(self.outputs, outs):
            net.vars[v].value = t

    def backward(self, net):
        r = self.rec
        douts = [net.vars[v].der for v in self.outputs]
        if all(d is None for d in douts):
            return
        dins, dpar = self._derivatives(net, [net.vars[v].value for v in r.inputs], douts)
        for v, d in zip(r.inputs, dins):
            net._set_var_der(v, d)
        for p, d in zip(r.params, dpar):
            net._set_param_der(p, d)
        for v in self.outputs:
            _release_der(net, net.vars[v])


class _ConvStep(_Step):

    reads_through_conv = True

    def __init__(self, rec):
        super().__init__(rec)
        self.bias_from = None
        self.moments_for = None
        self.stem_into = None

    def forward(self, net):
        if self.stem_into is not None and self.stem_into.stem_forward(net, self):
            return
        super().forward(net)

    def _values(self, net, ins):
        r, blk = self.rec, self.rec.block
        prm = self._params(net)
        if net._training and net.wgradStream is not None and net.vars[r.inputs[0]].fanin > 0 and net.prepareBackward:
            with torch.cuda.stream(net.wgradStream):
                vl.conv_prepare_backward(ins[0], prm[0], stride=blk.stride, pad=blk.pad, dilate=blk.dilate)
        bn = self.moments_for
        if bn is not None and net._training and net.mode != "test" and net.fuseStats:
            do = net._direct_der(bn)
            mo = do[2] if do else vl.mat_empty(bn.block.numChannels, 2, device=ins[0].device)
            y = vl.vl_nnconv(ins[0], prm[0], prm[1] if blk.hasBias else None, stride=blk.stride, pad=blk.pad,
                             dilate=blk.dilate, moments_out=mo, epsilon=bn.block.epsilon)
            bn.block._pre_moments = mo
            return [y]
        if self.precision is not None:
            return [_forward_conv(self, ins[0], prm[0], prm[1] if blk.hasBias else None, stride=self._stride(), pad=blk.pad,
                                  dilate=blk.dilate)]
        if self.run_stride is not None:
            return [vl.vl_nnconv(ins[0], prm[0], prm[1] if blk.hasBias else None, stride=self.run_stride, pad=blk.pad,
                                 dilate=blk.dilate)]
        return blk.forward(ins, prm)

    def _derivatives(self, net, ins, douts):
        r = self.rec
        need_dx = net.vars[r.inputs[0]].fanin > 0
        skip_db = self.bias_from is not None and self.bias_from.bias_conv_done
        side = net.wgradStream if need_dx else None
        if side is not None and net._flat is not None and net._direct_der(r) is None:
            side = None
        xin = net.vars[r.inputs[0]]
        accum = xin.der if need_dx else None
        if accum is not None:
            xin.der = None
        if side is None:
            dins, dpar = r.block.backward(ins, self._params(net), douts, need_dx=need_dx,
                                          der_out=net._direct_der(r), skip_db=skip_db, dx_accum=accum)
            if net.gradHook is not None:
                if net._side_pending:
                    torch.cuda.current_stream().wait_stream(net.wgradStream)
                net.gradHook(r.name)
        else:
            main = torch.cuda.current_stream()
            defer = net.wgradAfterDgrad
            if defer:
                dins, _ = r.block.backward(ins, self._params(net), douts, need_dx=True, need_df=False,
                                           dx_accum=accum)
            side.wait_stream(main)
            with torch.cuda.stream(side):
                _, dpar = r.block.backward(ins, self._params(net), douts, need_dx=False,
                                           der_out=net._direct_der(r), skip_db=skip_db)
                if net.gradHook is not None:
                    net.gradHook(r.name)
            douts[0].record_stream(side)
            ins[0].record_stream(side)
            net._side_pending = True
            if not defer:
                dins, _ = r.block.backward(ins, self._params(net), douts, need_dx=True, need_df=False,
                                           dx_accum=accum)
        if skip_db:
            dpar = [dpar[0], net.params[r.params[1]].der]
        return dins, dpar


class _BnStep(_Step):

    bias_der_always = False
    relu = False

    def __init__(self, rec, *swallowed):
        super().__init__(rec, *swallowed)
        self.bias_conv = None
        self.bias_conv_done = False

    def take_bias_of(self, conv_step):
        self.bias_conv, conv_step.bias_from = conv_step, self

    def _bias_der_slot(self, net):
        self.bias_conv_done = False
        if self.bias_conv is None or net._flat is None or net.accumulateParamDers:
            return None
        if not self.bias_der_always and (not net.fuseBiasDer or net.wgradStream is not None):
            return None
        bp = net.params[self.bias_conv.rec.params[1]]
        if bp.fanout == 1 and bp.der is not None:
            self.bias_conv_done = True
            return bp.der
        return None

    def _values(self, net, ins):
        return self.rec.block.forward(ins, self._params(net), relu=self.relu)

    def _derivatives(self, net, ins, douts):
        y = net.vars[self.outputs[0]].value if self.relu else None
        return self.rec.block.backward(ins, self._params(net), douts, relu=self.relu, y=y,
                                       der_out=net._direct_der(self.rec), dxsum_out=self._bias_der_slot(net))


class _PoolStep(_Step):

    def _derivatives(self, net, ins, douts):
        outs = [net.vars[v].value for v in self.rec.outputs]
        return self.rec.block.backward(ins, self._params(net), douts, outputs=outs if outs[0] is not None else None)


class _GlobalPoolStep(_PoolStep):

    def __init__(self, rec):
        super().__init__(rec)
        self.se_bn = None

    def _values(self, net, ins):
        f = self.se_bn.fwd if self.se_bn is not None else None
        if f is None:
            return super()._values(net, ins)
        return [vl.se_squeeze_bn(f["u"], f["g"], f["b"], f["moments"])]

    def _derivatives(self, net, ins, douts):
        if self.se_bn is not None and self.se_bn.stash is not None:
            self.se_bn.stash["dgp"] = douts[0]
            return [], []
        xin = net.vars[self.rec.inputs[0]]
        if self.rec.block.method != "avg" or xin.der is None or not net.fuseForkSums:
            return super()._derivatives(net, ins, douts)
        acc, xin.der = xin.der, None
        return [vl.vl_nnpool(ins[0], [int(ins[0].shape[0]), int(ins[0].shape[1])], douts[0], method="avg",
                             dx_accum=acc)], []


class _BnReluStep(_BnStep):

    relu = True

    def __init__(self, bn_rec, relu_rec):
        super().__init__(bn_rec, relu_rec)
        self.relu_rec = relu_rec


class _AddReluStep(_Step):

    def __init__(self, rec, relu_rec):
        super().__init__(rec, relu_rec)
        self.relu_rec = relu_rec
        self.se_bn = None

    def _values(self, net, ins):
        if self.se_bn is not None and self.se_bn.fwd is not None:
            f = self.se_bn.fwd
            return [vl.scale_axpy_bn(f["u"], ins[0], ins[2], f["g"], f["b"], f["moments"], relu=True)]
        return self.rec.block.forward(ins, [], relu=True)

    def _derivatives(self, net, ins, douts):
        out = net.vars[self.outputs[0]]
        if self.se_bn is not None and self.se_bn.begin(net, out):
            return [], []
        dz = vl.vl_nnrelu(out.value, douts[0])
        return self.rec.block.backward(ins, [], [dz])


class _SEBnTrainStep(_BnStep):

    def __init__(self, bn_rec, axpy_rec, gp_rec):
        super().__init__(bn_rec)
        self.axpy_rec, self.gp_rec = axpy_rec, gp_rec
        self.stash = self.fwd = None

    def forward(self, net):
        r = self.rec
        self.fwd = None
        xv = net.vars[r.outputs[0]]
        if net.fuseSETrain and net._training and not xv.precious:
            g, b, mom = self._params(net)
            test = net.mode == "test"
            moments = mom if test else r.block.take_pre_moments()
            if moments is not None:
                r.block.moments = None if test else moments
                self.fwd = {"u": net.vars[r.inputs[0]].value, "g": g, "b": b, "moments": moments}
                xv.value = None
                return
        super().forward(net)

    def begin(self, net, out):
        self.stash = None
        self.bias_conv_done = False
        if not net.fuseSETrain:
            if self.fwd is not None:
                raise RuntimeError("fused SE tail: fuseSETrain was switched off between the forward and the backward pass")
            return False
        r, ax = self.rec, self.axpy_rec
        gate_v, x_v, sc_v = (net.vars[v] for v in ax.inputs)
        if x_v.precious or net.vars[r.outputs[0]] is not x_v:
            if self.fwd is not None:
                raise RuntimeError("fused SE tail: the forward pass skipped X but the fused backward cannot run (%s)" % r.name)
            return False
        g, b, mom = self._params(net)
        test = net.mode == "test"
        moments = mom if test else r.block.moments
        if moments is None:
            return False
        u = net.vars[r.inputs[0]].value
        da, sums = vl.se_tail_backward_reduce(out.value, out.der, u, g, b, moments)
        net._set_var_der(ax.inputs[0], da)
        self.stash = {"y": out.value, "dzdy": out.der, "u": u, "sums": sums, "gate": gate_v.value, "moments": moments,
                      "test": test, "shortcut": ax.inputs[2], "dgp": None}
        return True

    def backward(self, net):
        st, self.stash = self.stash, None
        if st is None:
            return super().backward(net)
        r = self.rec
        if st["dgp"] is None:
            raise RuntimeError("fused SE tail: the squeeze's derivative never arrived (layer %s)" % r.name)
        g, b, mom = self._params(net)
        do = net._direct_der(r)
        dz, du, dg, db = vl.se_tail_backward_apply(st["y"], st["dzdy"], st["u"], st["gate"], st["dgp"], g, st["moments"],
                                                   st["sums"], train=not st["test"], dg_out=do[0] if do else None,
                                                   db_out=do[1] if do else None)
        net._set_var_der(st["shortcut"], dz)
        net._set_var_der(r.inputs[0], du)
        for p, d in zip(r.params, [dg, db, None if st["test"] else st["moments"]]):
            net._set_param_der(p, d)


class _BnReluPoolStep(_BnStep):

    bias_der_always = True

    def __init__(self, bn_rec, relu_rec, pool_rec):
        super().__init__(bn_rec, relu_rec, pool_rec)
        self.relu_rec, self.pool_rec = relu_rec, pool_rec
        self._saved = None
        self.producer_conv = None
        self._stem_fused = True
        self._stem_fwd_ok = True
        self._stem_fwd = None

    def _stem_conditions(self, net):
        cs = self.producer_conv
        if cs is None or net._flat is None or net.accumulateParamDers:
            return None
        cr, r = cs.rec, self.rec
        if net.vars[cr.inputs[0]].fanin > 0 or net.vars[cr.outputs[0]].precious:
            return None
        do, cdo = net._direct_der(r), net._direct_der(cr)
        if do is None or cdo is None or any(net.params[p].fanout != 1 for p in cr.params):
            return None
        return cs, do, cdo

    def stem_forward(self, net, cs):
        self._stem_fwd = None
        if not (self._stem_fwd_ok and self._stem_fused and net.fuseStemForward and net.fuseStemGram and
                net.fuseStemBackward and net._training and net.fuseStats):
            return False
        ok = self._stem_conditions(net)
        if ok is None or ok[0] is not cs:
            return False
        _, do, _ = ok
        r, pb, blk = self.rec, self.pool_rec.block, cs.rec.block
        g, b, mom = self._params(net)
        test = net.mode == "test"
        cpar = cs._params(net)
        res = vl.conv_bnorm_relu_pool(net.vars[cs.rec.inputs[0]].value, cpar[0], cpar[1] if blk.hasBias else None, g, b,
                                      pb.poolSize, stride=blk.stride, pad=blk.pad, dilate=blk.dilate, pool_stride=pb.stride,
                                      pool_pad=pb.pad, epsilon=r.block.epsilon, moments=mom if test else None,
                                      moments_out=None if test else do[2])
        if res is None:
            self._stem_fwd_ok = False
            return False
        y, am, mo, gram = res
        r.block.moments = None if test else mo
        self._saved = (am, mo)
        self._stem_fwd = {"gram": gram}
        net.vars[self.pool_rec.outputs[0]].value = y
        return True

    @staticmethod
    def eligible(pool_block):
        ph, pw = pool_block.poolSize
        sy, sx = vl._pair(pool_block.stride, "STRIDE")
        return pool_block.method == "max" and -(-ph // sy) <= 2 and -(-pw // sx) <= 2 and ph * pw <= 255

    def forward(self, net):
        if self._stem_fwd is not None:
            return
        r, pb = self.rec, self.pool_rec.block
        x = net.vars[r.inputs[0]].value
        g, b, mom = self._params(net)
        test = net.mode == "test"
# ... 168 lines not shown
            bn_ = vl.to_numpy(bias).astype(np.float64).ravel() if bias is not None else np.zeros(Cc)
            f10 = (Fm * scn[None, :]) @ F1m
            b10 = F1m.T @ (scn * bn_ + shn)
            if b1 is not None:
                b10 = b10 + vl.to_numpy(b1).astype(np.float64).ravel()
            self._reduce = (key,
                            vl.from_numpy(np.asfortranarray(f10.astype(np.float32).reshape(1, 1, Kp, -1, order="F")), F.device),
                            vl.from_numpy(b10.astype(np.float32).reshape(-1, 1), F.device))
        return self._reduce[1], self._reduce[2]

    def _values(self, net, ins):
        blk, se, u = self.rec.block, self.se, ins[0]
        prm = self._params(net)
        bias = prm[1] if blk.hasBias else None
        sc, sh = self._fold(net)
        ubar = vl.vl_nnpool(u, [int(u.shape[0]), int(u.shape[1])], method="avg")
        f1 = [net.params[p].value for p in se["fc1"].params]
        f2 = [net.params[p].value for p in se["fc2"].params]
        b1 = f1[1] if se["fc1"].block.hasBias else None
        if net.foldSEReduce:
            f10, b10 = self._fold_reduce(net, prm[0], bias, sc, sh, f1[0], b1)
            h = vl.vl_nnconv(ubar, f10, b10, relu=True)
        else:
            z = vl.vl_nnconv(ubar, prm[0], bias, scale=sc, shift=sh)
            h = vl.vl_nnconv(z, f1[0], b1, relu=True)
        a = vl.vl_nnconv(h, f2[0], f2[1] if se["fc2"].block.hasBias else None, sigmoid=True)
        return [_forward_conv(self, u, prm[0], bias, stride=self._stride(), pad=blk.pad, dilate=blk.dilate, scale=sc, shift=sh,
                              gate=a, residual=net.vars[se["shortcut"]].value, residual_stride=self.run_stride,
                              relu=se["relu"] is not None)]


class _Wiring:

    def __init__(self, net):
        self.net = net
        self.order = {id(r): i for i, r in enumerate(net.layers)}
        self.consumers, self.producers = {}, {}
        for r in net.layers:
            for v in r.inputs:
                self.consumers.setdefault(v, []).append(r)
            for v in r.outputs:
                self.producers.setdefault(v, []).append(r)

    def sole_consumer(self, var, cls, keep_value=False):
        cs = self.consumers.get(var, [])
        ok = len(cs) == 1 and isinstance(cs[0].block, cls) and (keep_value or not self.net.vars[var].precious)
        return cs[0] if ok else None

    def fused_relu(self, var, keep_value=False):
        rl = self.sole_consumer(var, ReLU, keep_value)
        return rl if rl is not None and rl.block.leak == 0.0 else None

    def produced_before(self, var, rec):
        return all(self.order[id(q)] < self.order[id(rec)] for q in self.producers.get(var, ()))

    def feeding_conv(self, rec):
        var = rec.inputs[0]
        prod = self.producers.get(var, [])
        ok = prod and isinstance(prod[0].block, Conv) and len(self.consumers.get(var, [])) == 1
        return prod[0] if ok else None


def _conv_1x1(blk, unit_stride=False, unit_dilate=True):
    return isinstance(blk, Conv) and blk.size[0] == 1 and blk.size[1] == 1 and not any(vl._pad4(blk.pad)) and \
        (not unit_stride or tuple(vl._pair(blk.stride, "STRIDE")) == (1, 1)) and \
        (not unit_dilate or tuple(vl._pair(blk.dilate, "DILATE")) == (1, 1))


def _match_se_tail(w, conv_rec, bn_rec, keep_values=False):
    if not _conv_1x1(conv_rec.block, unit_stride=True, unit_dilate=False):
        return None
    x = bn_rec.outputs[0]
    cs = w.consumers.get(x, [])
    if len(cs) != 2 or w.net.vars[x].precious:
        return None
    gp = [c for c in cs if isinstance(c.block, GlobalPooling) and c.block.method == "avg"]
    ax = [c for c in cs if isinstance(c.block, Axpy)]
    if len(gp) != 1 or len(ax) != 1:
        return None
    gp, ax = gp[0], ax[0]
    fc1 = w.sole_consumer(gp.outputs[0], Conv, keep_values)
    r1 = w.sole_consumer(fc1.outputs[0], ReLU, keep_values) if fc1 else None
    fc2 = w.sole_consumer(r1.outputs[0], Conv, keep_values) if r1 else None
    sg = w.sole_consumer(fc2.outputs[0], Sigmoid, keep_values) if fc2 else None
    if sg is None or r1.block.leak != 0.0 or w.sole_consumer(sg.outputs[0], Axpy, keep_values) is not ax:
        return None
    if not all(_conv_1x1(fc.block, unit_stride=True, unit_dilate=False) for fc in (fc1, fc2)):
        return None
    if len(ax.inputs) != 3 or ax.inputs[0] != sg.outputs[0] or ax.inputs[1] != x:
        return None
    shortcut = ax.inputs[2]
    if not w.produced_before(shortcut, conv_rec):
        return None
    return {"gp": gp, "fc1": fc1, "relu1": r1, "fc2": fc2, "sig": sg, "axpy": ax,
            "relu": w.fused_relu(ax.outputs[0], keep_values), "shortcut": shortcut}


def _fold_forward_only(w, r):
    if not isinstance(r.block, Conv):
        return None
    bn = w.sole_consumer(r.outputs[0], BatchNorm)
    if bn is None:
        act = w.sole_consumer(r.outputs[0], (ReLU, Sigmoid))
        if act is not None and (isinstance(act.block, Sigmoid) or act.block.leak == 0.0):
            return _ConvActStep(r, act)
        return None
    se = _match_se_tail(w, r, bn) if w.net.fuseSE else None
    if se is not None:
        return _SEFoldStep(r, bn, se)
    out = bn.outputs[0]
    sm = w.sole_consumer(out, Sum)
    if sm is not None and len(sm.inputs) == 2 and w.produced_before([v for v in sm.inputs if v != out][0], r):
        out = sm.outputs[0]
    else:
        sm = None
    return _ConvFoldStep(r, bn, sm, w.fused_relu(out))


def _fuse_common(w, r):
    if isinstance(r.block, Axpy) or (isinstance(r.block, Sum) and len(r.inputs) == 2):
        rl = w.fused_relu(r.outputs[0])
        return _AddReluStep(r, rl) if rl is not None else None
    if isinstance(r.block, BatchNorm):
        rl = w.fused_relu(r.outputs[0])
        pl = w.sole_consumer(rl.outputs[0], Pooling) if rl is not None else None
        if pl is not None and not isinstance(pl.block, GlobalPooling) and _BnReluPoolStep.eligible(pl.block):
            return _BnReluPoolStep(r, rl, pl)
        return _BnReluStep(r, rl) if rl is not None else None
    return None


def _se_train_head(w, r):
    conv = w.feeding_conv(r) if isinstance(r.block, BatchNorm) else None
    se = _match_se_tail(w, conv, r, keep_values=True) if conv is not None else None
    if se is None or w.fused_relu(se["axpy"].outputs[0]) is None:
        return None
    return _SEBnTrainStep(r, se["axpy"], se["gp"])


def _unfused(r):
    for cls, step in ((Conv, _ConvStep), (BatchNorm, _BnStep), (GlobalPooling, _GlobalPoolStep), (Pooling, _PoolStep)):
        if isinstance(r.block, cls):
            return step(r)
    return _Step(r)


def _link_training(w, steps):
    by_rec = {id(st.rec): st for st in steps}
    for st in steps:
        if isinstance(st, _SEBnTrainStep):
            ax, gp = by_rec[id(st.axpy_rec)], by_rec[id(st.gp_rec)]
            assert type(ax) is _AddReluStep and type(gp) is _GlobalPoolStep, st.rec.name
            ax.se_bn = gp.se_bn = st
        conv = w.feeding_conv(st.rec) if isinstance(st, _BnStep) else None
        if conv is None:
            continue
        cs = by_rec[id(conv)]
        assert isinstance(cs, _ConvStep), conv.name
        cs.moments_for = st.rec
        if conv.block.hasBias:
            st.take_bias_of(cs)
        if isinstance(st, _BnReluPoolStep):
            st.producer_conv, cs.stem_into = cs, st


def _prune_strided_boundaries(w, steps):
    head = {id(st.rec): st for st in steps}
    for st in steps:
        if not isinstance(st, _ConvFoldStep) or st.run_stride is not None or \
                not _conv_1x1(st.rec.block, unit_stride=True) or w.net.vars[st.outputs[0]].precious:
            continue
        readers = [head.get(id(c)) for c in w.consumers.get(st.outputs[0], [])]
        if not readers or any(q is None or not q.reads_through_conv or not _conv_1x1(q.rec.block) or
                              q.run_stride is not None for q in readers):
            continue
        strides = {tuple(vl._pair(q.rec.block.stride, "STRIDE")) for q in readers}
        if len(strides) != 1:
            continue
        s = strides.pop()
        if s[0] != s[1] or s[0] <= 1:
            continue
        st.run_stride = s
        for q in readers:
            q.run_stride = (1, 1)


def _prune_reader_lattices(w, steps):
    head = {id(st.rec): st for st in steps}
    for st in steps:
        if type(st) is not _ConvFoldStep or st.sum_rec is not None or st.run_stride is not None or \
                tuple(vl._pair(st.rec.block.stride, "STRIDE")) != (1, 1) or w.net.vars[st.outputs[0]].precious:
            continue
        readers = [head.get(id(c)) for c in w.consumers.get(st.outputs[0], [])]
        if len(readers) != 1 or readers[0] is None or not readers[0].reads_through_conv:
            continue
        s = readers[0].run_stride
        if s is None or s[0] != s[1] or s[0] <= 1 or not _conv_1x1(readers[0].rec.block, unit_stride=True):
            continue
        st.out_lattice = tuple(s)


def build_plan(net, training):
    w = _Wiring(net)
    fold = net.fuse and not training and net.mode == "test"
    steps, taken = [], set()
    for r in net.layers:
        if id(r) in taken:
            continue
        st = _fold_forward_only(w, r) if fold else None
        if st is None and net.fuse:
            st = _fuse_common(w, r) or (_se_train_head(w, r) if training else None)
        steps.append(st or _unfused(r))
        taken.update(id(q) for q in steps[-1].recs[1:])
    if net.fuse and training:
        _link_training(w, steps)
    if fold and net.stridePrune:
        _prune_strided_boundaries(w, steps)
        if net.latticePrune:
            _prune_reader_lattices(w, steps)
    if not training and net.mode == "test" and net.convPrecision == "bf16x3":
        for st in steps:
            if isinstance(st, (_ConvStep, _ConvActStep, _ConvFoldStep)):
                st.precision = "bf16x3"
    return steps
```

mcncrossmodalemotions_amd/vl.py:

```python
import ctypes as C

import numpy as np
import torch

from . import _lib



def _dev():
    return torch.device("cuda", torch.cuda.current_device())


XM_ENOTSUP = 5


def mat_empty(*shape, device=None):
    shape = tuple(int(s) for s in (shape[0] if len(shape) == 1 and not np.isscalar(shape[0]) else shape))
    t = torch.empty(tuple(reversed(shape)), dtype=torch.float32, device=device or _dev())
    return t.permute(*reversed(range(len(shape))))


def mat_zeros(*shape, device=None):
    t = mat_empty(*shape, device=device)
    t.zero_()
# ... 225 lines not shown
    L = _L()
    Ho, Wo = L.xm_out_size(H, pt, pb, FH, dy, sy), L.xm_out_size(W, pl, pr, FW, dx, sx)
    for name, v in (("SCALE", scale), ("SHIFT", shift)):
        if v is not None and _chk(v, name).numel() != K:
            raise ValueError("vl_nnconv: %s has %d elements, expected %d" % (name, v.numel(), K))
    gt = None
    if gate is not None:
        gt = _chk(gate, "GATE")
        if gt.numel() != K * N:
            raise ValueError("vl_nnconv: GATE must be 1 x 1 x %d x %d" % (K, N))
    RH, RW, rsy, rsx = 0, 0, 1, 1
    if residual_stride is not None and residual is None:
        raise ValueError("vl_nnconv: residual_stride without a residual")
    if residual is not None:
        RH, RW, RK, RN = _shape4(_chk(residual, "RESIDUAL"))
        if residual_stride is not None:
            rsy, rsx = _pair(residual_stride, "RESIDUAL_STRIDE")
        if [RK, RN] != [K, N] or (residual_stride is None and [RH, RW] != [Ho, Wo]):
            raise ValueError("vl_nnconv: residual shape mismatch")
    y = mat_empty(max(Ho, 0), max(Wo, 0), K, N, device=x.device)
    _lib.check(L.xm_nnconv_forward_split(
        _ptr(x), H, W, Cc, N, _ptr(f), FH, FW, FC, K, _ptr(bb), _ptr(y), sy, sx, pt, pb, pl, pr, dy, dx,
        _ptr(scale), _ptr(shift), _ptr(gt), _ptr(residual), RH, RW, rsy, rsx, 1 if relu else 0, CONV_BF16X3, _stream()))
    return y


def conv_prepare_backward(x, f, stride=1, pad=0, dilate=1):
    H, W, Cc, N = _shape4(x)
    FH, FW, FC, K = _shape4(f)
    sy, sx = _pair(stride, "STRIDE")
    dy, dx = _pair(dilate, "DILATE")
    pt, pb, pl, pr = _pad4(pad)
    _lib.check(_L().xm_nnconv_prepare_backward(H, W, Cc, N, _ptr(f), FH, FW, FC, K, sy, sx, pt, pb, pl, pr, dy, dx,
                                               _stream()))


def params_changed():
    _lib.check(_L().xm_params_changed())


_METHOD = {"max": 0, "avg": 1}


def vl_nnpool(x, pool, dzdy=None, stride=1, pad=0, method="max", argmax=None, want_argmax=False, dx_accum=None):
    x = _chk(x, "X")
    if method not in _METHOD:
        raise ValueError("vl_nnpool: unknown METHOD '%s'" % method)
    H, W, Cc, N = _shape4(x)
    ph, pw = _pair(pool, "POOL")
    sy, sx = _pair(stride, "STRIDE")
    pt, pb, pl, pr = _pad4(pad)
    L = _L()
    Ho = L.xm_out_size(H, pt, pb, ph, 1, sy)
    Wo = L.xm_out_size(W, pl, pr, pw, 1, sx)
    if dzdy is None:
        y = mat_empty(max(Ho, 0), max(Wo, 0), Cc, N, device=x.device)
        if want_argmax and method == "max":
            am = torch.empty(max(Ho, 0) * max(Wo, 0) * Cc * N, dtype=torch.uint8, device=x.device)
            _lib.check(L.xm_nnpool_forward_argmax(_ptr(x), H, W, Cc, N, ph, pw, sy, sx, pt, pb, pl, pr,
                                                  _ptr(y), C.c_void_p(am.data_ptr()), _stream()))
            return y, am
        _lib.check(L.xm_nnpool_forward(_ptr(x), H, W, Cc, N, ph, pw, sy, sx, pt, pb, pl, pr,
                                       _METHOD[method], _ptr(y), _stream()))
        return (y, None) if want_argmax else y
    dzdy = _chk(dzdy, "DZDY")
    if _shape4(dzdy) != [Ho, Wo, Cc, N]:
        raise ValueError("vl_nnpool: DZDY is %r, expected %r" % (tuple(dzdy.shape), (Ho, Wo, Cc, N)))
    dxo = mat_empty(H, W, Cc, N, device=x.device)
    if dx_accum is not None:
        if method != "avg" or (ph, pw) != (H, W) or (pt | pb | pl | pr) or _shape4(dx_accum) != [H, W, Cc, N]:
            raise ValueError("vl_nnpool: dx_accum is built for global average pooling only")
        _lib.check(L.xm_nnpool_global_avg_backward_accum(_ptr(dzdy), _ptr(_chk(dx_accum, "DX_ACCUM")), _ptr(dxo), H, W, Cc, N,
                                                         _stream()))
        return dxo
    if argmax is not None and method == "max":
        _lib.check(L.xm_nnpool_backward_argmax(C.c_void_p(argmax.data_ptr()), H, W, Cc, N, ph, pw, sy,
                                               sx, pt, pb, pl, pr, _ptr(dzdy), _ptr(dxo), _stream()))
    else:
        _lib.check(L.xm_nnpool_backward(_ptr(x), H, W, Cc, N, ph, pw, sy, sx, pt, pb, pl, pr,
                                        _METHOD[method], _ptr(dzdy), _ptr(dxo), _stream()))
    return dxo




def vl_nnbnorm(x, g, b, dzdy=None, epsilon=1e-4, moments=None, relu=False, y=None, dg_out=None,
               db_out=None, moments_out=None, batch_moments=False, dxsum_out=None):
    x, g, b = _chk(x, "X"), _chk(g, "G"), _chk(b, "B")
    H, W, Cc, N = _shape4(x)
    if g.numel() != Cc or b.numel() != Cc:
        raise ValueError("vl_nnbnorm: G and B must have %d elements" % Cc)
    mi = None
    if moments is not None:
        mi = _chk(moments, "MOMENTS")
        if mi.numel() != 2 * Cc:
            raise ValueError("vl_nnbnorm: MOMENTS must be %d x 2" % Cc)
    L = _L()
    mo = moments_out if moments_out is not None else mat_empty(Cc, 2, device=x.device)
    if dzdy is None:
        yo = mat_empty(H, W, Cc, N, device=x.device)
        _lib.check(L.xm_nnbnorm_forward_fused(_ptr(x), H, W, Cc, N, _ptr(g), _ptr(b),
                                              float(epsilon), _ptr(mi), _ptr(yo), _ptr(mo),
                                              1 if relu else 0, _stream()))
        return yo, mo
    dzdy = _chk(dzdy, "DZDY")
    if _shape4(dzdy) != [H, W, Cc, N]:
        raise ValueError("vl_nnbnorm: DZDY shape mismatch")
    dxo = mat_empty(H, W, Cc, N, device=x.device)
    dg = dg_out if dg_out is not None else mat_empty(Cc, 1, device=x.device)
    db = db_out if db_out is not None else mat_empty(Cc, 1, device=x.device)
    if batch_moments and mi is None:
        raise ValueError("vl_nnbnorm: batch_moments needs the moments of the forward call")
    if dxsum_out is not None:
        if relu and y is None:
            raise ValueError("vl_nnbnorm: fused backward needs the forward output y")
        if _chk(dxsum_out, "DXSUM").numel() != Cc:
            raise ValueError("vl_nnbnorm: dxsum_out must have %d elements" % Cc)
        _lib.check(L.xm_nnbnorm_backward_dxsum(_ptr(x), _ptr(_chk(y, "Y")) if relu else None, H, W, Cc, N,
                                               _ptr(g), _ptr(b), _ptr(dzdy), float(epsilon), _ptr(mi),
                                               _ptr(dxo), _ptr(dg), _ptr(db), _ptr(mo), _ptr(dxsum_out),
                                               (1 if relu else 0) | (2 if batch_moments else 0), _stream()))
    elif relu or batch_moments:
        if relu and y is None:
            raise ValueError("vl_nnbnorm: fused backward needs the forward output y")
        _lib.check(L.xm_nnbnorm_backward_fused(_ptr(x), _ptr(_chk(y, "Y")) if relu else None, H, W, Cc, N,
                                               _ptr(g), _ptr(b), _ptr(dzdy), float(epsilon), _ptr(mi),
                                               _ptr(dxo), _ptr(dg), _ptr(db), _ptr(mo),
                                               (1 if relu else 0) | (2 if batch_moments else 0), _stream()))
    else:
        _lib.check(L.xm_nnbnorm_backward(_ptr(x), H, W, Cc, N, _ptr(g), _ptr(b), _ptr(dzdy),
                                         float(epsilon), _ptr(mi), _ptr(dxo), _ptr(dg), _ptr(db),
                                         _ptr(mo), _stream()))
    return dxo, dg, db, mo


def bnorm_relu_pool(x, g, b, pool, stride=1, pad=0, epsilon=1e-4, moments=None, moments_out=None):
    x, g, b = _chk(x, "X"), _chk(g, "G"), _chk(b, "B")
    H, W, Cc, N = _shape4(x)
    ph, pw = _pair(pool, "POOL")
    sy, sx = _pair(stride, "STRIDE")
    pt, pb, pl, pr = _pad4(pad)
    L = _L()
    Ho, Wo = L.xm_out_size(H, pt, pb, ph, 1, sy), L.xm_out_size(W, pl, pr, pw, 1, sx)
    y = mat_empty(max(Ho, 0), max(Wo, 0), Cc, N, device=x.device)
    am = torch.empty(max(Ho, 0) * max(Wo, 0) * Cc * N, dtype=torch.uint8, device=x.device)
    mo = moments_out if moments_out is not None else mat_empty(Cc, 2, device=x.device)
    mi = None if moments is None else _chk(moments, "MOMENTS")
    _lib.check(L.xm_nnbnorm_relu_pool_forward(_ptr(x), H, W, Cc, N, _ptr(g), _ptr(b), float(epsilon),
                                              _ptr(mi), ph, pw, sy, sx, pt, pb, pl, pr, _ptr(y),
                                              C.c_void_p(am.data_ptr()), _ptr(mo), _stream()))
    return y, am, mo


def bnorm_relu_pool_backward(x, g, b, moments, argmax, dzdy, pool, stride=1, pad=0, train=True,
                             dg_out=None, db_out=None, need_dx=True, dxsum_out=None, y_pool=None):
    x, g, b, dzdy = _chk(x, "X"), _chk(g, "G"), _chk(b, "B"), _chk(dzdy, "DZDY")
    H, W, Cc, N = _shape4(x)
    ph, pw = _pair(pool, "POOL")
    sy, sx = _pair(stride, "STRIDE")
    pt, pb, pl, pr = _pad4(pad)
    dx = mat_empty(H, W, Cc, N, device=x.device) if need_dx else None
    dg = dg_out if dg_out is not None else mat_empty(Cc, 1, device=x.device)
    db = db_out if db_out is not None else mat_empty(Cc, 1, device=x.device)
    _lib.check(_L().xm_nnbnorm_relu_pool_backward(
        _ptr(x), H, W, Cc, N, _ptr(g), _ptr(b), _ptr(_chk(moments, "MOMENTS")), 1 if train else 0, ph, pw,
        sy, sx, pt, pb, pl, pr, C.c_void_p(argmax.data_ptr()),
        None if y_pool is None else _ptr(_chk(y_pool, "Y_POOL")), _ptr(dzdy), _ptr(dx), _ptr(dg), _ptr(db),
        _ptr(dxsum_out), _stream()))
    return dx, dg, db


def conv_backward_filter_bnrelupool(x, filter_shape, y, g, b, moments, argmax, y_pool, dzdy, pool, stride=1, pad=0,
                                    dilate=1, pool_stride=1, pool_pad=0, train=True, df_out=None, dbias_out=None,
                                    dg_out=None, db_out=None, has_bias=True):
    x, y, g, b, dzdy = _chk(x, "X"), _chk(y, "Y"), _chk(g, "G"), _chk(b, "B"), _chk(dzdy, "DZDY")
    H, W, Cc, N = _shape4(x)
    FH, FW, FC, K = (int(v) for v in filter_shape)
    sy, sx = _pair(stride, "STRIDE")
    dy, dx = _pair(dilate, "DILATE")
    pt, pb, pl, pr = _pad4(pad)
    ph, pw = _pair(pool, "POOL")
    psy, psx = _pair(pool_stride, "STRIDE")
    ppt, ppb, ppl, ppr = _pad4(pool_pad)
    df = df_out if df_out is not None else mat_empty(FH, FW, FC, K, device=x.device)
    dbias = (dbias_out if dbias_out is not None else mat_empty(K, 1, device=x.device)) if has_bias else None
    dg = dg_out if dg_out is not None else mat_empty(K, 1, device=x.device)
    db = db_out if db_out is not None else mat_empty(K, 1, device=x.device)
    rc = _L().xm_nnconv_backward_filter_bnrelupool(
        _ptr(x), H, W, Cc, N, FH, FW, FC, K, sy, sx, pt, pb, pl, pr, dy, dx, _ptr(y), _ptr(g), _ptr(b),
        _ptr(_chk(moments, "MOMENTS")), 1 if train else 0, ph, pw, psy, psx, ppt, ppb, ppl, ppr,
        C.c_void_p(argmax.data_ptr()), None if y_pool is None else _ptr(_chk(y_pool, "Y_POOL")), _ptr(dzdy), _ptr(df),
        _ptr(dbias), _ptr(dg), _ptr(db), _stream())
    if rc == XM_ENOTSUP:
        return None
    _lib.check(rc)
    return df, dbias, dg, db


def stem_gram(x, filter_shape, stride=1, pad=0):
    x = _chk(x, "X")
    H, W, Cc, N = _shape4(x)
    FH, FW = int(filter_shape[0]), int(filter_shape[1])
    sy, sx = _pair(stride, "STRIDE")
    pt, pb, pl, pr = _pad4(pad)
    if Cc != 1:
        return None
    gram = torch.empty(64 * 64, dtype=torch.float64, device=x.device)
    rc = _L().xm_stem_gram(_ptr(x), H, W, N, FH, FW, sy, sx, pt, pb, pl, pr, C.c_void_p(gram.data_ptr()), _stream())
    if rc == XM_ENOTSUP:
        return None
    _lib.check(rc)
    return gram


def stem_gram_moments(gram, f, b, epsilon=1e-4, moments_out=None):
    f = _chk(f, "F")
    FH, FW, FC, K = _shape4(f)
    mo = moments_out if moments_out is not None else mat_empty(K, 2, device=f.device)
    _lib.check(_L().xm_stem_gram_moments(C.c_void_p(gram.data_ptr()), _ptr(f), _ptr(None if b is None else _chk(b, "B")),
                                         FH, FW, K, float(epsilon), _ptr(mo), _stream()))
    return mo


def conv_bnorm_relu_pool(x, f, bias, g, b, pool, stride=1, pad=0, dilate=1, pool_stride=1, pool_pad=0, epsilon=1e-4,
                         moments=None, moments_out=None, gram=None):
    x, f, g, b = _chk(x, "X"), _chk(f, "F"), _chk(g, "G"), _chk(b, "B")
    H, W, Cc, N = _shape4(x)
    FH, FW, FC, K = _shape4(f)
    sy, sx = _pair(stride, "STRIDE")
    dy, dx = _pair(dilate, "DILATE")
    pt, pb, pl, pr = _pad4(pad)
    ph, pw = _pair(pool, "POOL")
    psy, psx = _pair(pool_stride, "STRIDE")
    ppt, ppb, ppl, ppr = _pad4(pool_pad)
    L = _L()
    Ho, Wo = L.xm_out_size(H, pt, pb, FH, dy, sy), L.xm_out_size(W, pl, pr, FW, dx, sx)
    pHo, pWo = L.xm_out_size(Ho, ppt, ppb, ph, 1, psy), L.xm_out_size(Wo, ppl, ppr, pw, 1, psx)
    if Ho <= 0 or Wo <= 0 or pHo <= 0 or pWo <= 0:
        return None
    y = mat_empty(pHo, pWo, K, N, device=x.device)
    am = torch.empty(pHo * pWo * K * N, dtype=torch.uint8, device=x.device)
    mi = None if moments is None else _chk(moments, "MOMENTS")
    mo = None
    if mi is None:
        mo = moments_out if moments_out is not None else mat_empty(K, 2, device=x.device)
        if gram is None:
            gram = torch.empty(64 * 64, dtype=torch.float64, device=x.device)
    rc = L.xm_nnconv_bnorm_relu_pool_forward(
        _ptr(x), H, W, Cc, N, _ptr(f), FH, FW, FC, K, None if bias is None else _ptr(_chk(bias, "B")), sy, sx, pt, pb, pl, pr,
        dy, dx, _ptr(g), _ptr(b), float(epsilon), _ptr(mi), ph, pw, psy, psx, ppt, ppb, ppl, ppr,
        None if gram is None else C.c_void_p(gram.data_ptr()), _ptr(y), C.c_void_p(am.data_ptr()), _ptr(mo), _stream())
    if rc == XM_ENOTSUP:
        return None
    _lib.check(rc)
    return y, am, (mi if mo is None else mo), gram


def conv_backward_filter_bnrelupool_gram(x, f, bias, g, moments, argmax, y_pool, dzdy, pool, stride=1, pad=0, dilate=1,
                                         pool_stride=1, pool_pad=0, train=True, gram=None, df_out=None, dbias_out=None,
                                         dg_out=None, db_out=None):
    x, f, g, dzdy = _chk(x, "X"), _chk(f, "F"), _chk(g, "G"), _chk(dzdy, "DZDY")
    H, W, Cc, N = _shape4(x)
    FH, FW, FC, K = _shape4(f)
    sy, sx = _pair(stride, "STRIDE")
    dy, dx = _pair(dilate, "DILATE")
    pt, pb, pl, pr = _pad4(pad)
    ph, pw = _pair(pool, "POOL")
    psy, psx = _pair(pool_stride, "STRIDE")
    ppt, ppb, ppl, ppr = _pad4(pool_pad)
    has_bias = bias is not None
    df = df_out if df_out is not None else mat_empty(FH, FW, FC, K, device=x.device)
    dbias = (dbias_out if dbias_out is not None else mat_empty(K, 1, device=x.device)) if has_bias else None
    dg = dg_out if dg_out is not None else mat_empty(K, 1, device=x.device)
    db = db_out if db_out is not None else mat_empty(K, 1, device=x.device)
    rc = _L().xm_nnconv_backward_filter_bnrelupool_gram(
        _ptr(x), H, W, Cc, N, _ptr(f), FH, FW, FC, K, _ptr(_chk(bias, "B")) if has_bias else None, sy, sx, pt, pb, pl, pr,
        dy, dx, _ptr(g), _ptr(_chk(moments, "MOMENTS")), 1 if train else 0, ph, pw, psy, psx, ppt, ppb, ppl, ppr,
        C.c_void_p(argmax.data_ptr()), None if y_pool is None else _ptr(_chk(y_pool, "Y_POOL")), _ptr(dzdy),
        None if gram is None else C.c_void_p(gram.data_ptr()), _ptr(df), _ptr(dbias), _ptr(dg), _ptr(db), _stream())
    if rc == XM_ENOTSUP:
        return None
    _lib.check(rc)
    return df, dbias, dg, db




def vl_nnrelu(x, dzdy=None, leak=0.0):
    x = _chk(x, "X")
    y = mat_empty(*x.shape, device=x.device)
    d = None if dzdy is None else _chk(dzdy, "DZDY")
    _lib.check(_L().xm_nnrelu(_ptr(x), x.numel(), float(leak), _ptr(d), _ptr(y), _stream()))
    return y


def nnnormalize_geometry():
    v = [C.c_int(0) for _ in range(3)]
    _lib.check(_L().xm_nnnormalize_geometry(*[C.byref(t) for t in v]))
    return tuple(int(t.value) for t in v)


def vl_nnnormalize(x, param, dzdy=None, out=None):
    x = _chk(x, "X")
    param = [float(v) for v in np.asarray(param, dtype=np.float64).ravel()]
    if len(param) != 4:
        raise ValueError("PARAM must have four elements [N KAPPA ALPHA BETA]")
# ... 1125 lines not shown
```

Measured before the change: 4180 pairs/s.

## Fuse batch-norm, ReLU and global average pool into one head kernel

Adds a single-pass head kernel that computes per-channel batch moments, applies BN+ReLU, and optionally global-average-pools within one wave per channel, with a matching fused backward. A lazy conv-moments entry point lets the conv skip its separate moment reduction when the following head step will compute the moments itself. This is meant to remove the separate moments, normalize, relu and pool launches and their intermediate tensor traffic in the student's small final layers. It adds graph-matching logic between BN/ReLU and pooling steps, plus an env switch to fall back to the composed operators.

```diff
diff --git a/include/xmodal.h b/include/xmodal.h
--- a/include/xmodal.h
+++ b/include/xmodal.h
@@ -71,6 +71,10 @@
 int xm_nnconv_forward_moments(const float *x, int H, int W, int C, int N, const float *f, int FH, int FW,
                               int FC, int K, const float *b, float *y, int sy, int sx, int pt, int pb,
                               int pl, int pr, int dy, int dx, float epsilon, float *moments_out, void *stream);
+int xm_nnconv_forward_moments_lazy(const float *x, int H, int W, int C, int N, const float *f, int FH, int FW,
+                                   int FC, int K, const float *b, float *y, int sy, int sx, int pt, int pb,
+                                   int pl, int pr, int dy, int dx, float epsilon, float *moments_out, int *computed,
+                                   void *stream);
 int xm_nnconv_backward(const float *x, int H, int W, int C, int N, const float *f, int FH, int FW,
                        int FC, int K, const float *dzdy, float *dx_out, float *df_out,
                        float *db_out, int sy, int sx, int pt, int pb, int pl, int pr, int dy,
@@ -150,6 +154,13 @@
                                   const unsigned char *argmax, const float *y_pool, const float *dzdy_pool,
                                   float *dx_out, float *dg_out, float *db_out, float *dxsum_out, void *stream);
 
+int xm_nnbnorm_relu_head_geometry(int H, int W, int C, int N, int pool, int *quads);
+int xm_nnbnorm_relu_head_forward(const float *x, int H, int W, int C, int N, const float *g, const float *b,
+                                 float epsilon, float *y, float *y_pool, float *moments_out, void *stream);
+int xm_nnbnorm_relu_head_backward(const float *x, int H, int W, int C, int N, const float *g, const float *b,
+                                  const float *moments, int pool, const float *dzdy, float *dx_out, float *dg_out,
+                                  float *db_out, float *dxsum_out, void *stream);
+
 int xm_nnrelu(const float *x, size_t n, float leak, const float *dzdy, float *y, void *stream);
 int xm_nnsigmoid(const float *x, size_t n, const float *dzdy, float *y, void *stream);
 int xm_sum2(const float *a, const float *b, size_t n, int flags, float *y, void *stream);
diff --git a/mcncrossmodalemotions_amd/_lib.py b/mcncrossmodalemotions_amd/_lib.py
--- a/mcncrossmodalemotions_amd/_lib.py
+++ b/mcncrossmodalemotions_amd/_lib.py
@@ -29,6 +29,8 @@
     "xm_out_size": [_i] * 6,
     "xm_nnconv_forward": [c_fp] + [_i] * 4 + [c_fp] + [_i] * 4 + [c_fp, c_fp] + [_i] * 8 + [_vp],
     "xm_nnconv_forward_moments": [c_fp] + [_i] * 4 + [c_fp] + [_i] * 4 + [c_fp, c_fp] + [_i] * 8 + [_f, c_fp, _vp],
+    "xm_nnconv_forward_moments_lazy": [c_fp] + [_i] * 4 + [c_fp] + [_i] * 4 + [c_fp, c_fp] + [_i] * 8 +
+                                      [_f, c_fp, C.POINTER(C.c_int), _vp],
     "xm_nnconv_forward_gated": [c_fp] + [_i] * 4 + [c_fp] + [_i] * 4 + [c_fp, c_fp] + [_i] * 8 +
                                [c_fp, c_fp, c_fp, c_fp, _i, _vp],
     "xm_nnconv_forward_strided_residual": [c_fp] + [_i] * 4 + [c_fp] + [_i] * 4 + [c_fp, c_fp] + [_i] * 8 +
@@ -71,6 +73,9 @@
                                     [c_fp, c_fp, c_fp, _vp],
     "xm_nnbnorm_relu_pool_backward": [c_fp] + [_i] * 4 + [c_fp, c_fp, c_fp, _i] + [_i] * 8 +
                                      [c_fp, c_fp, c_fp, c_fp, c_fp, c_fp, c_fp, _vp],
+    "xm_nnbnorm_relu_head_geometry": [_i] * 5 + [C.POINTER(C.c_int)],
+    "xm_nnbnorm_relu_head_forward": [c_fp] + [_i] * 4 + [c_fp, c_fp, _f, c_fp, c_fp, c_fp, _vp],
+    "xm_nnbnorm_relu_head_backward": [c_fp] + [_i] * 4 + [c_fp, c_fp, c_fp, _i, c_fp, c_fp, c_fp, c_fp, c_fp, _vp],
     "xm_nndropout_forward": [c_fp, _sz, _f, C.c_ulonglong, C.c_ulonglong, c_fp, c_fp, _vp],
     "xm_nndropout_apply": [c_fp, c_fp, _sz, c_fp, _vp],
     "xm_nnrelu": [c_fp, _sz, _f, c_fp, c_fp, _vp],
diff --git a/mcncrossmodalemotions_amd/build.py b/mcncrossmodalemotions_amd/build.py
--- a/mcncrossmodalemotions_amd/build.py
+++ b/mcncrossmodalemotions_amd/build.py
@@ -7,8 +7,8 @@
 CSRC = os.path.join(HERE, "csrc")
 TAG = os.environ.get("XM_BUILD_TAG", "")
 OUT = os.path.join(HERE, "libxmodal_hip%s.so" % ("_" + TAG if TAG else ""))
-SOURCES = ["context.cpp", "prof.cpp", "conv.hip", "conv_split.hip", "stem_pool.hip", "norm_pool.hip", "lrn.hip", "misc.hip", "spec.hip", "sampler.hip", "eval.hip", "roc.hip", "imdb.hip", "jpeg.hip", "jpeg_prog.hip", "wav.hip", "pixcsv.hip", "comm.cpp"]
-HEADERS = ["xm_common.h", "fastdiv.h", "prof.h", "conv_plan.h", "stem_pool_plan.h", "conv_split_plan.h", "norm_pool_plan.h", "conv_tune.h", "wav_plan.h", "wav_resample.h", "pixcsv_plan.h", "jpeg_scan_plan.h", "jpeg_entropy.h", "conv_kernels.h", "stem_pool_kernels.h", os.path.join("..", "..", "include", "xmodal.h")]
+SOURCES = ["context.cpp", "prof.cpp", "conv.hip", "conv_split.hip", "stem_pool.hip", "norm_pool.hip", "fc_head.hip", "lrn.hip", "misc.hip", "spec.hip", "sampler.hip", "eval.hip", "roc.hip", "imdb.hip", "jpeg.hip", "jpeg_prog.hip", "wav.hip", "pixcsv.hip", "comm.cpp"]
+HEADERS = ["xm_common.h", "fastdiv.h", "prof.h", "conv_plan.h", "stem_pool_plan.h", "conv_split_plan.h", "norm_pool_plan.h", "fc_head_plan.h", "conv_tune.h", "wav_plan.h", "wav_resample.h", "pixcsv_plan.h", "jpeg_scan_plan.h", "jpeg_entropy.h", "conv_kernels.h", "stem_pool_kernels.h", os.path.join("..", "..", "include", "xmodal.h")]
 FLAGS = ["--offload-arch=gfx950", "-O3", "-std=c++17", "-fPIC", "-Wall", "-Wno-unused-function"]
 if os.environ.get("XM_DEBUG_CYCLES"):
     FLAGS.append("-DXM_DEBUG_CYCLES")
diff --git a/mcncrossmodalemotions_amd/csrc/context.cpp b/mcncrossmodalemotions_amd/csrc/context.cpp
--- a/mcncrossmodalemotions_amd/csrc/context.cpp
+++ b/mcncrossmodalemotions_amd/csrc/context.cpp
@@ -18,6 +18,10 @@
     read = true;
   }
   return on[p];
+}
+bool fc_head_on() {
+  static const bool on = getenv("XM_NO_FC_HEAD") == nullptr;
+  return on;
 }
 
 long long env_int(const char *name, long long dflt) {
@@ -94,7 +98,7 @@
 
 extern "C" {
 
-int xm_version(void) { return 124; }
+int xm_version(void) { return 125; }
 const char *xm_last_error(void) { return xm::err_buf(); }
 
 int xm_workspace_reserve(size_t bytes) {
diff --git a/mcncrossmodalemotions_amd/csrc/conv.hip b/mcncrossmodalemotions_amd/csrc/conv.hip
--- a/mcncrossmodalemotions_amd/csrc/conv.hip
+++ b/mcncrossmodalemotions_amd/csrc/conv.hip
@@ -1145,7 +1145,7 @@
 static int conv_forward(const float *x, const float *f, const float *b, float *y, const Geo &g,
                         const float *scale, const float *shift, const float *resid, int relu,
                         hipStream_t st, float *moments_out = nullptr, float eps = 0.f, const float *gate = nullptr,
-                        int res_H = 0, int res_W = 0, int res_sy = 1, int res_sx = 1) {
+                        int res_H = 0, int res_W = 0, int res_sy = 1, int res_sx = 1, bool *moments_done = nullptr) {
   const bool padded = (g.pt | g.pb | g.pl | g.pr) != 0;
   const bool bigTaps = g.FH * g.FW > 63;
   if (bigTaps && padded)
@@ -1193,7 +1193,8 @@
       stats_done = true;
     }
   }
-  if (moments_out && !stats_done) return bn_batch_moments(y, g.Ho, g.Wo, g.K, g.N, eps, moments_out, st);
+  if (moments_done) *moments_done = stats_done;
+  if (moments_out && !stats_done && !moments_done) return bn_batch_moments(y, g.Ho, g.Wo, g.K, g.N, eps, moments_out, st);
   return XM_OK;
 }
 
@@ -2061,6 +2062,26 @@
   return conv_forward(x, f, b, y, g, nullptr, nullptr, nullptr, 0, st, moments_out, epsilon);
 }
 
+int xm_nnconv_forward_moments_lazy(const float *x, int H, int W, int C, int N, const float *f, int FH, int FW,
+                                   int FC, int K, const float *b, float *y, int sy, int sx, int pt, int pb,
+                                   int pl, int pr, int dy, int dx, float epsilon, float *moments_out, int *computed,
+                                   void *stream) {
+  Geo g;
+  int rc = make_geo(g, H, W, C, N, FH, FW, FC, K, sy, sx, pt, pb, pl, pr, dy, dx);
+  if (rc) return rc;
+  if (!x || !f || !y || !moments_out || !computed) return fail(XM_EINVAL, "vl_nnconv(+moments): NULL tensor");
+  hipStream_t st = (hipStream_t)stream;
+  *computed = 0;
+  if (fc_skinny_ok(g)) {
+    g_last_stats_splits = 0;
+    return fc_skinny_forward(x, f, b, y, g, 0, st);
+  }
+  bool done = false;
+  rc = conv_forward(x, f, b, y, g, nullptr, nullptr, nullptr, 0, st, moments_out, epsilon, nullptr, 0, 0, 1, 1, &done);
+  *computed = done ? 1 : 0;
+  return rc;
+}
+
 int xm_nnconv_forward_gated(const float *x, int H, int W, int C, int N, const float *f, int FH, int FW,
                             int FC, int K, const float *b, float *y, int sy, int sx, int pt, int pb,
                             int pl, int pr, int dy, int dx, const float *scale, const float *shift,
diff --git a/mcncrossmodalemotions_amd/csrc/fc_head.hip b/mcncrossmodalemotions_amd/csrc/fc_head.hip
--- /dev/null
+++ b/mcncrossmodalemotions_amd/csrc/fc_head.hip
@@ -0,0 +1,243 @@
+#include "fc_head_plan.h"
+#include "norm_pool_plan.h"
+#include "prof.h"
+#include "xm_common.h"
+
+namespace xm {
+
+__device__ __forceinline__ float bn_head_pre(float sc, float mu, float bb, float v) { return __fmaf_rn(sc, v - mu, bb); }
+
+template <bool VEC>
+__device__ __forceinline__ size_t bn_head_item(int j, int c, int HW, int C, int run, FastDiv divRun, int &n) {
+  n = (int)xm_div((uint32_t)j, divRun);
+  const int r = j - n * run;
+  return (size_t)HW * (c + (size_t)C * n) + (size_t)(VEC ? 4 * r : r);
+}
+
+template <bool VEC, int E>
+__device__ __forceinline__ void bn_head_load(const float *__restrict__ p, float (&v)[E]) {
+  if constexpr (VEC) {
+    const float4 q = *reinterpret_cast<const float4 *>(p);
+    v[0] = q.x, v[1] = q.y, v[2] = q.z, v[3] = q.w;
+  } else {
+    v[0] = *p;
+  }
+}
+template <bool VEC, int E>
+__device__ __forceinline__ void bn_head_store(float *__restrict__ p, const float (&v)[E]) {
+  if constexpr (VEC)
+    *reinterpret_cast<float4 *>(p) = make_float4(v[0], v[1], v[2], v[3]);
+  else
+    *p = v[0];
+}
+template <bool VEC, int E>
+__device__ __forceinline__ float bn_head_sum(const float (&v)[E]) {
+  if constexpr (VEC)
+    return (v[0] + v[1]) + (v[2] + v[3]);
+  else
+    return v[0];
+}
+
+template <bool VEC, bool POOL>
+__global__ void __launch_bounds__(256)
+bn_head_fwd_kernel(const float *__restrict__ x, const float *__restrict__ g, const float *__restrict__ b,
+                   float *__restrict__ y, float *__restrict__ yp, float *__restrict__ mom, int HW, int C, int N, int items,
+                   int run, FastDiv divRun, float eps, float inv_hw) {
+  constexpr int IT = VEC ? kHeadLaneItems / 4 : kHeadLaneItems, E = VEC ? 4 : 1;
+  const int c = blockIdx.x * 4 + (threadIdx.x >> 6), lane = threadIdx.x & 63;
+  if (c >= C) return;
+  const float shift = x[(size_t)HW * c];
+  float v[IT][E];
+  size_t off[IT];
+  int smp[IT];
+  double a = 0.0, s2 = 0.0;
+#pragma unroll
+  for (int i = 0; i < IT; ++i) {
+    const int j = lane + 64 * i;
+    off[i] = 0, smp[i] = 0;
+#pragma unroll
+    for (int e = 0; e < E; ++e) v[i][e] = shift;
+    if (j < items) {
+      off[i] = bn_head_item<VEC>(j, c, HW, C, run, divRun, smp[i]);
+      bn_head_load<VEC>(x + off[i], v[i]);
+    }
+#pragma unroll
+    for (int e = 0; e < E; ++e) {
+      const double d = (double)v[i][e] - (double)shift;
+      a += d;
+      s2 += d * d;
+    }
+  }
+  a = xm_wave_sum_d(a);
+  s2 = xm_wave_sum_d(s2);
+  const double m = (double)HW * N, d = a / m;
+  double var = s2 / m - d * d;
+  var = var < 0.0 ? 0.0 : var;
+  const float mu = (float)((double)shift + d), sg = (float)sqrt(var + (double)eps);
+  if (lane == 0) {
+    mom[c] = mu;
+    mom[C + c] = sg;
+  }
+  const float sc = g[c] / sg, bb = b[c];
+#pragma unroll
+  for (int i = 0; i < IT; ++i) {
+    const bool ok = lane + 64 * i < items;
+    float o[E];
+#pragma unroll
+    for (int e = 0; e < E; ++e) o[e] = fmaxf(bn_head_pre(sc, mu, bb, v[i][e]), 0.f);
+    if (ok && y) bn_head_store<VEC>(y + off[i], o);
+    if (POOL) {
+      float s = bn_head_sum<VEC>(o);
+      for (int w = run >> 1; w > 0; w >>= 1) s += __shfl_xor(s, w, 64);
+      if (ok && (lane & (run - 1)) == 0) yp[c + (size_t)C * smp[i]] = s * inv_hw;
+    }
+  }
+}
+
+template <bool VEC, bool POOL>
+__global__ void __launch_bounds__(256)
+bn_head_bwd_kernel(const float *__restrict__ x, const float *__restrict__ dzdy, const float *__restrict__ g,
+                   const float *__restrict__ b, const float *__restrict__ mom, float *__restrict__ dx,
+                   float *__restrict__ dg, float *__restrict__ db, float *__restrict__ dxsum, int HW, int C, int N,
+                   int items, int run, FastDiv divRun, float inv_hw) {
+  constexpr int IT = VEC ? kHeadLaneItems / 4 : kHeadLaneItems, E = VEC ? 4 : 1;
+  const int c = blockIdx.x * 4 + (threadIdx.x >> 6), lane = threadIdx.x & 63;
+  if (c >= C) return;
+  const float muf = mom[c], sgf = mom[C + c], gc = g[c];
+  const float sc = gc / sgf, bb = b[c];
+  const double mu = muf, sg = sgf;
+  float v[IT][E], dz[IT][E];
+  size_t off[IT];
+  double a = 0.0, s2 = 0.0;
+#pragma unroll
+  for (int i = 0; i < IT; ++i) {
+    const int j = lane + 64 * i;
+    off[i] = 0;
+#pragma unroll
+    for (int e = 0; e < E; ++e) v[i][e] = muf, dz[i][e] = 0.f;
+    if (j < items) {
+      int n;
+      off[i] = bn_head_item<VEC>(j, c, HW, C, run, divRun, n);
+      bn_head_load<VEC>(x + off[i], v[i]);
+      if (POOL) {
+        const float t = dzdy[c + (size_t)C * n] * inv_hw;
+#pragma unroll
+        for (int e = 0; e < E; ++e) dz[i][e] = t;
+      } else {
+        bn_head_load<VEC>(dzdy + off[i], dz[i]);
+      }
+#pragma unroll
+      for (int e = 0; e < E; ++e) {
+        if (!(bn_head_pre(sc, muf, bb, v[i][e]) > 0.f)) dz[i][e] = 0.f;
+        a += (double)dz[i][e];
+        s2 += (double)dz[i][e] * ((double)v[i][e] - mu);
+      }
+    }
+  }
+  a = xm_wave_sum_d(a);
+  s2 = xm_wave_sum_d(s2);
+  const double m = (double)HW * N, gs = (double)gc / sg, c1 = a / m, c2 = s2 / (m * sg * sg);
+  double acc = 0.0;
+#pragma unroll
+  for (int i = 0; i < IT; ++i) {
+    if (lane + 64 * i < items) {
+      float o[E];
+#pragma unroll
+      for (int e = 0; e < E; ++e) {
+        o[e] = (float)(gs * ((double)dz[i][e] - c1 - ((double)v[i][e] - mu) * c2));
+        acc += (double)o[e];
+      }
+      bn_head_store<VEC>(dx + off[i], o);
+    }
+  }
+  if (dxsum) acc = xm_wave_sum_d(acc);
+  if (lane == 0) {
+    dg[c] = (float)(s2 / sg);
+    db[c] = (float)a;
+    if (dxsum) dxsum[c] = (float)acc;
+  }
+}
+
+static int head_geo(int H, int W, int C, int N, bool pool, HeadPlan &p) {
+  if (H <= 0 || W <= 0 || C <= 0 || N <= 0) return fail(XM_EINVAL, "vl_nnbnorm(head): empty tensor");
+  if (too_big(H, W, C, N)) return fail(XM_ETOOBIG, "vl_nnbnorm(head): tensor with >= 2^31 elements");
+  p = head_plan(H, W, C, N, pool);
+  if (!p.can || !fc_head_on())
+    return fail(XM_ENOTSUP, "vl_nnbnorm(head): %d x %d x %d x %d%s is left to the composed operators", H, W, C, N,
+                pool ? " (pooled)" : "");
+  return XM_OK;
+}
+
+}
+
+using namespace xm;
+
+extern "C" {
+
+int xm_nnbnorm_relu_head_geometry(int H, int W, int C, int N, int pool, int *quads) {
+  const HeadPlan p = head_plan(H, W, C, N, pool != 0);
+  if (quads) *quads = p.can && p.quads ? 1 : 0;
+  return p.can && fc_head_on() ? 1 : 0;
+}
+
+int xm_nnbnorm_relu_head_forward(const float *x, int H, int W, int C, int N, const float *g, const float *b,
+                                 float epsilon, float *y, float *y_pool, float *moments_out, void *stream) {
+  HeadPlan p;
+  int rc = head_geo(H, W, C, N, y_pool != nullptr, p);
+  if (rc) return rc;
+  if (!x || !g || !b || !moments_out || (!y && !y_pool)) return fail(XM_EINVAL, "vl_nnbnorm(head): NULL tensor");
+  hipStream_t st = (hipStream_t)stream;
+  const int HW = H * W;
+  const bool vec = p.quads && aligned16(x, y);
+  const int items = head_items(HW, N, vec), run = head_run(HW, vec);
+  const FastDiv dr = make_fastdiv((uint32_t)run);
+  const float inv = 1.0f / (float)HW;
+  ProfScope ps(prof_key(kProfFcHead, (y_pool ? 2 : 0) + (vec ? 1 : 0)), 0, st,
+               4.0 * ((double)HW * C * N * (y ? 2 : 1) + (y_pool ? (double)C * N : 0.0) + 4.0 * C));
+#define XM_HEAD_FWD(V, P) \
+  hipLaunchKernelGGL((bn_head_fwd_kernel<V, P>), dim3(p.blocks), dim3(256), 0, st, x, g, b, y, y_pool, moments_out, HW, C, N, \
+                     items, run, dr, epsilon, inv)
+  if (y_pool) {
+    if (vec) XM_HEAD_FWD(true, true);
+    else XM_HEAD_FWD(false, true);
+  } else {
+    if (vec) XM_HEAD_FWD(true, false);
+    else XM_HEAD_FWD(false, false);
+  }
+#undef XM_HEAD_FWD
+  XM_LAUNCH_CHECK();
+  return XM_OK;
+}
+
+int xm_nnbnorm_relu_head_backward(const float *x, int H, int W, int C, int N, const float *g, const float *b,
+                                  const float *moments, int pool, const float *dzdy, float *dx_out, float *dg_out,
+                                  float *db_out, float *dxsum_out, void *stream) {
+  HeadPlan p;
+  int rc = head_geo(H, W, C, N, pool != 0, p);
+  if (rc) return rc;
+  if (!x || !g || !b || !moments || !dzdy || !dx_out || !dg_out || !db_out)
+    return fail(XM_EINVAL, "vl_nnbnorm(head): NULL tensor");
+  hipStream_t st = (hipStream_t)stream;
+  const int HW = H * W;
+  const bool vec = p.quads && aligned16(x, dx_out) && (pool || aligned16(dzdy));
+  const int items = head_items(HW, N, vec), run = head_run(HW, vec);
+  const FastDiv dr = make_fastdiv((uint32_t)run);
+  const float inv = 1.0f / (float)HW;
+  ProfScope ps(prof_key(kProfFcHead, 4 + (pool ? 2 : 0) + (vec ? 1 : 0)), 0, st,
+               4.0 * ((double)HW * C * N * (pool ? 2 : 3) + (pool ? (double)C * N : 0.0) + 7.0 * C));
+#define XM_HEAD_BWD(V, P) \
+  hipLaunchKernelGGL((bn_head_bwd_kernel<V, P>), dim3(p.blocks), dim3(256), 0, st, x, dzdy, g, b, moments, dx_out, dg_out, \
+                     db_out, dxsum_out, HW, C, N, items, run, dr, inv)
+  if (pool) {
+    if (vec) XM_HEAD_BWD(true, true);
+    else XM_HEAD_BWD(false, true);
+  } else {
+    if (vec) XM_HEAD_BWD(true, false);
+    else XM_HEAD_BWD(false, false);
+  }
+#undef XM_HEAD_BWD
+  XM_LAUNCH_CHECK();
+  return XM_OK;
+}
+
+}
diff --git a/mcncrossmodalemotions_amd/csrc/fc_head_plan.h b/mcncrossmodalemotions_amd/csrc/fc_head_plan.h
--- /dev/null
+++ b/mcncrossmodalemotions_amd/csrc/fc_head_plan.h
@@ -0,0 +1,34 @@
+#pragma once
+#include <cstddef>
+#include <cstdint>
+
+namespace xm {
+
+constexpr int kHeadLaneItems = 8;
+constexpr int kHeadMaxValues = 64 * kHeadLaneItems;
+constexpr int kHeadMaxPlain = 32;
+
+struct HeadPlan {
+  bool can;
+  bool quads;
+  int blocks;
+};
+inline HeadPlan head_plan(int H, int W, int C, int N, bool pool) {
+  HeadPlan p{false, false, 0};
+  if (H <= 0 || W <= 0 || C <= 0 || N <= 0) return p;
+  const long long HW = (long long)H * W, m = HW * N;
+  if (m > (pool ? kHeadMaxValues : kHeadMaxPlain) || m * C >= (1ll << 31)) return p;
+  if (pool && (HW > 64 || (HW & (HW - 1)) != 0)) return p;
+  p.can = true;
+  p.quads = (HW & 3) == 0;
+  p.blocks = (C + 3) / 4;
+  return p;
+}
+inline int head_items(int HW, int N, bool vec) { return vec ? (HW >> 2) * N : HW * N; }
+inline int head_run(int HW, bool vec) { return vec ? HW >> 2 : HW; }
+inline size_t head_offset(int HW, int C, int c, int j, bool vec) {
+  const int run = head_run(HW, vec), n = j / run, i = j - n * run;
+  return (size_t)HW * (c + (size_t)C * n) + (size_t)(vec ? 4 * i : i);
+}
+
+}
diff --git a/mcncrossmodalemotions_amd/csrc/prof.cpp b/mcncrossmodalemotions_amd/csrc/prof.cpp
--- a/mcncrossmodalemotions_amd/csrc/prof.cpp
+++ b/mcncrossmodalemotions_amd/csrc/prof.cpp
@@ -34,7 +34,7 @@
 struct ProfRow {
   ProfKind kind;
   int nsub;
-  const char *names[6];
+  const char *names[8];
 };
 static const ProfRow kProfRows[] = {
     {kProfGemm, 2 * 12, {}},
@@ -60,6 +60,9 @@
     {kProfWavRate, 2, {"wav_rate_gain_kernel", "wav_resample_kernel"}},
     {kProfPixcsv, 1, {"pixcsv_decode_kernel"}},
     {kProfConvSplit, 1, {"conv_split_kernel"}},
+    {kProfFcHead, 8, {"bn_head_fwd_kernel<false, false>", "bn_head_fwd_kernel<true, false>", "bn_head_fwd_kernel<false, true>",
+                      "bn_head_fwd_kernel<true, true>", "bn_head_bwd_kernel<false, false>", "bn_head_bwd_kernel<true, false>",
+                      "bn_head_bwd_kernel<false, true>", "bn_head_bwd_kernel<true, true>"}},
     {kProfLrn, 6, {"lrn_forward_kernel<5, false>", "lrn_forward_kernel<5, true>", "lrn_backward_kernel<5, false>",
                    "lrn_backward_kernel<5, true>", "lrn_general_kernel<false>", "lrn_general_kernel<true>"}},
 };
diff --git a/mcncrossmodalemotions_amd/csrc/prof.h b/mcncrossmodalemotions_amd/csrc/prof.h
--- a/mcncrossmodalemotions_amd/csrc/prof.h
+++ b/mcncrossmodalemotions_amd/csrc/prof.h
@@ -26,6 +26,7 @@
   kProfJpegProg = 26,
   kProfWavRate = 27,
   kProfConvSplit = 28,
+  kProfFcHead = 29,
 };
 constexpr int prof_key(ProfKind kind, int sub = 0) { return kind * 100 + sub; }
 
diff --git a/mcncrossmodalemotions_amd/csrc/xm_common.h b/mcncrossmodalemotions_amd/csrc/xm_common.h
--- a/mcncrossmodalemotions_amd/csrc/xm_common.h
+++ b/mcncrossmodalemotions_amd/csrc/xm_common.h
@@ -72,6 +72,7 @@
   kPathCount
 };
 bool path_on(Path p);
+bool fc_head_on();
 long long env_int(const char *name, long long dflt);
 double env_double(const char *name, double dflt);
 
diff --git a/mcncrossmodalemotions_amd/dagnn.py b/mcncrossmodalemotions_amd/dagnn.py
--- a/mcncrossmodalemotions_amd/dagnn.py
+++ b/mcncrossmodalemotions_amd/dagnn.py
@@ -816,7 +816,9 @@
         super().__init__(rec)
         self.bias_from = None
         self.moments_for = None
+        self.moments_step = None
         self.stem_into = None
+        self._head_ok = {}
 
     def forward(self, net):
         if self.stem_into is not None and self.stem_into.stem_forward(net, self):
@@ -833,6 +835,11 @@
         if bn is not None and net._training and net.mode != "test" and net.fuseStats:
             do = net._direct_der(bn)
             mo = do[2] if do else vl.mat_empty(bn.block.numChannels, 2, device=ins[0].device)
+            if self._head_takes_moments(ins[0], prm[0]):
+                y, done = vl.conv_moments_lazy(ins[0], prm[0], prm[1] if blk.hasBias else None, mo, stride=blk.stride,
+                                               pad=blk.pad, dilate=blk.dilate, epsilon=bn.block.epsilon)
+                bn.block._pre_moments = mo if done else None
+                return [y]
             y = vl.vl_nnconv(ins[0], prm[0], prm[1] if blk.hasBias else None, stride=blk.stride, pad=blk.pad,
                              dilate=blk.dilate, moments_out=mo, epsilon=bn.block.epsilon)
             bn.block._pre_moments = mo
@@ -844,6 +851,19 @@
             return [vl.vl_nnconv(ins[0], prm[0], prm[1] if blk.hasBias else None, stride=self.run_stride, pad=blk.pad,
                                  dilate=blk.dilate)]
         return blk.forward(ins, prm)
+
+    def _head_takes_moments(self, x, f):
+        hs = self.moments_step
+        if not isinstance(hs, _BnReluStep):
+            return False
+        key = (tuple(x.shape), tuple(f.shape))
+        got = self._head_ok.get(key)
+        if got is None:
+            blk = self.rec.block
+            Ho, Wo = vl.conv_out_size(x, f, stride=blk.stride, pad=blk.pad, dilate=blk.dilate)
+            got = self._head_ok[key] = Ho > 0 and Wo > 0 and \
+                hs.head_covers((Ho, Wo, vl._shape4(f)[3], vl._shape4(x)[3]))[0]
+        return got
 
     def _derivatives(self, net, ins, douts):
         r = self.rec
@@ -922,6 +942,27 @@
 
 class _PoolStep(_Step):
 
+    def __init__(self, rec):
+        super().__init__(rec)
+        self.head_bn = None
+
+    def covers_plane(self, H, W):
+        blk = self.rec.block
+        return blk.method == "avg" and [int(v) for v in blk.poolSize] == [H, W] and not any(vl._pad4(blk.pad))
+
+    def forward(self, net):
+        if self.head_bn is not None and self.head_bn.head_pooled():
+            return
+        super().forward(net)
+
+    def backward(self, net):
+        if self.head_bn is not None and self.head_bn.head_pooled():
+            out = net.vars[self.outputs[0]]
+            self.head_bn.take_pool_der(out.der)
+            _release_der(net, out)
+            return
+        super().backward(net)
+
     def _derivatives(self, net, ins, douts):
         outs = [net.vars[v].value for v in self.rec.outputs]
         return self.rec.block.backward(ins, self._params(net), douts, outputs=outs if outs[0] is not None else None)
@@ -958,6 +999,64 @@
     def __init__(self, bn_rec, relu_rec):
         super().__init__(bn_rec, relu_rec)
         self.relu_rec = relu_rec
+        self.head_pool = None
+        self._head = None
+        self._head_geo = {}
+
+    def head_covers(self, shape):
+        got = self._head_geo.get(tuple(shape))
+        if got is None:
+            H, W, C, N = (int(v) for v in shape)
+            pooled = self.head_pool is not None and self.head_pool.covers_plane(H, W) and \
+                vl.bnorm_relu_head_covers(H, W, C, N, pool=True)
+            got = self._head_geo[tuple(shape)] = (pooled or vl.bnorm_relu_head_covers(H, W, C, N), pooled)
+        return got
+
+    def head_pooled(self):
+        return self._head is not None and self._head["pool"]
+
+    def take_pool_der(self, d):
+        self._head["dpool"] = d
+
+    def forward(self, net):
+        self._head = None
+        r = self.rec
+        x = net.vars[r.inputs[0]].value
+        if net._training and net.mode != "test":
+            runs, pooled = self.head_covers(vl._shape4(x))
+            if runs:
+                g, b, _ = self._params(net)
+                do = net._direct_der(r)
+                pre = r.block.take_pre_moments()
+                res = vl.bnorm_relu_head(x, g, b, epsilon=r.block.epsilon, pool=pooled,
+                                         moments_out=pre if pre is not None else (do[2] if do else None))
+                if res is not None:
+                    y, mo = res
+                    r.block.moments = mo
+                    self._head = {"pool": pooled, "mo": mo, "dpool": None}
+                    net.vars[self.head_pool.outputs[0] if pooled else self.outputs[0]].value = y
+                    return
+                r.block._pre_moments = pre
+        super().forward(net)
+
+    def backward(self, net):
+        h, self._head = self._head, None
+        if h is None:
+            return super().backward(net)
+        r = self.rec
+        out = net.vars[self.outputs[0]]
+        dz = h["dpool"] if h["pool"] else out.der
+        if dz is None:
+            return
+        g, b, _ = self._params(net)
+        do = net._direct_der(r)
+        dx, dg, db = vl.bnorm_relu_head_backward(net.vars[r.inputs[0]].value, g, b, h["mo"], dz, pool=h["pool"],
+                                                 dg_out=do[0] if do else None, db_out=do[1] if do else None,
+                                                 dxsum_out=self._bias_der_slot(net))
+        net._set_var_der(r.inputs[0], dx)
+        for p, d in zip(r.params, [dg, db, h["mo"]]):
+            net._set_param_der(p, d)
+        _release_der(net, out)
 
 
 class _AddReluStep(_Step):
@@ -1432,12 +1531,17 @@
             ax, gp = by_rec[id(st.axpy_rec)], by_rec[id(st.gp_rec)]
             assert type(ax) is _AddReluStep and type(gp) is _GlobalPoolStep, st.rec.name
             ax.se_bn = gp.se_bn = st
+        if isinstance(st, _BnReluStep):
+            pl = w.sole_consumer(st.outputs[0], Pooling)
+            ps = by_rec.get(id(pl)) if pl is not None and pl.block.method == "avg" else None
+            if type(ps) is _PoolStep:
+                st.head_pool, ps.head_bn = ps, st
         conv = w.feeding_conv(st.rec) if isinstance(st, _BnStep) else None
         if conv is None:
             continue
         cs = by_rec[id(conv)]
         assert isinstance(cs, _ConvStep), conv.name
-        cs.moments_for = st.rec
+        cs.moments_for, cs.moments_step = st.rec, st
         if conv.block.hasBias:
             st.take_bias_of(cs)
         if isinstance(st, _BnReluPoolStep):
diff --git a/mcncrossmodalemotions_amd/vl.py b/mcncrossmodalemotions_amd/vl.py
--- a/mcncrossmodalemotions_amd/vl.py
+++ b/mcncrossmodalemotions_amd/vl.py
@@ -401,6 +401,72 @@
     return y, am, mo
 
 
+def conv_out_size(x, f, stride=1, pad=0, dilate=1):
+    sy, sx = _pair(stride, "STRIDE")
+    dy, dx = _pair(dilate, "DILATE")
+    pt, pb, pl, pr = _pad4(pad)
+    L = _L()
+    return (L.xm_out_size(int(x.shape[0]), pt, pb, int(f.shape[0]), dy, sy),
+            L.xm_out_size(int(x.shape[1]), pl, pr, int(f.shape[1]), dx, sx))
+
+
+def conv_moments_lazy(x, f, b, moments_out, stride=1, pad=0, dilate=1, epsilon=1e-4):
+    x, f, mo = _chk(x, "X"), _chk(f, "F"), _chk(moments_out, "MOMENTS")
+    H, W, Cc, N = _shape4(x)
+    FH, FW, FC, K = _shape4(f)
+    sy, sx = _pair(stride, "STRIDE")
+    dy, dx = _pair(dilate, "DILATE")
+    pt, pb, pl, pr = _pad4(pad)
+    bb = None
+    if b is not None and b.numel() > 0:
+        bb = _chk(b, "B")
+        if bb.numel() != K:
+            raise ValueError("vl_nnconv: B has %d elements, expected %d" % (bb.numel(), K))
+    if mo.numel() != 2 * K:
+        raise ValueError("vl_nnconv: moments_out must be %d x 2" % K)
+    L = _L()
+    Ho, Wo = L.xm_out_size(H, pt, pb, FH, dy, sy), L.xm_out_size(W, pl, pr, FW, dx, sx)
+    y = mat_empty(max(Ho, 0), max(Wo, 0), K, N, device=x.device)
+    done = C.c_int(0)
+    _lib.check(L.xm_nnconv_forward_moments_lazy(_ptr(x), H, W, Cc, N, _ptr(f), FH, FW, FC, K, _ptr(bb), _ptr(y), sy, sx, pt, pb,
+                                                pl, pr, dy, dx, float(epsilon), _ptr(mo), C.byref(done), _stream()))
+    return y, bool(done.value)
+
+
+def bnorm_relu_head_covers(H, W, Cc, N, pool=False):
+    return _L().xm_nnbnorm_relu_head_geometry(int(H), int(W), int(Cc), int(N), 1 if pool else 0, None) == 1
+
+
+def bnorm_relu_head(x, g, b, epsilon=1e-4, pool=False, moments_out=None):
+    x, g, b = _chk(x, "X"), _chk(g, "G"), _chk(b, "B")
+    H, W, Cc, N = _shape4(x)
+    if g.numel() != Cc or b.numel() != Cc:
+        raise ValueError("vl_nnbnorm: G and B must have %d elements" % Cc)
+    if not bnorm_relu_head_covers(H, W, Cc, N, pool):
+        return None
+    y = mat_empty(1, 1, Cc, N, device=x.device) if pool else mat_empty(H, W, Cc, N, device=x.device)
+    mo = moments_out if moments_out is not None else mat_empty(Cc, 2, device=x.device)
+    _lib.check(_L().xm_nnbnorm_relu_head_forward(_ptr(x), H, W, Cc, N, _ptr(g), _ptr(b), float(epsilon),
+                                                 None if pool else _ptr(y), _ptr(y) if pool else None,
+                                                 _ptr(_chk(mo, "MOMENTS")), _stream()))
+    return y, mo
+
+
+def bnorm_relu_head_backward(x, g, b, moments, dzdy, pool=False, dg_out=None, db_out=None, dxsum_out=None):
+    x, g, b, dzdy = _chk(x, "X"), _chk(g, "G"), _chk(b, "B"), _chk(dzdy, "DZDY")
+    H, W, Cc, N = _shape4(x)
+    if _shape4(dzdy) != ([1, 1, Cc, N] if pool else [H, W, Cc, N]):
+        raise ValueError("vl_nnbnorm: DZDY shape mismatch")
+    if _chk(moments, "MOMENTS").numel() != 2 * Cc:
+        raise ValueError("vl_nnbnorm: MOMENTS must be %d x 2" % Cc)
+    dx = mat_empty(H, W, Cc, N, device=x.device)
+    dg = dg_out if dg_out is not None else mat_empty(Cc, 1, device=x.device)
+    db = db_out if db_out is not None else mat_empty(Cc, 1, device=x.device)
+    _lib.check(_L().xm_nnbnorm_relu_head_backward(_ptr(x), H, W, Cc, N, _ptr(g), _ptr(b), _ptr(moments), 1 if pool else 0,
+                                                  _ptr(dzdy), _ptr(dx), _ptr(dg), _ptr(db), _ptr(dxsum_out), _stream()))
+    return dx, dg, db
+
+
 def bnorm_relu_pool_backward(x, g, b, moments, argmax, dzdy, pool, stride=1, pad=0, train=True,
                              dg_out=None, db_out=None, need_dx=True, dxsum_out=None, y_pool=None):
     x, g, b, dzdy = _chk(x, "X"), _chk(g, "G"), _chk(b, "B"), _chk(dzdy, "DZDY")
```

Measured after the change: 4200 pairs/s (median of 3 runs). About the same (+0.5%).
